# eichenberger/stereo-svo-slam

Measured on AMD Instinct MI355X. Metric: tracked_frames_per_sec, higher is better.
Workload: dtype f32

## Files before the change

### include/svo_hip.h

```cpp
#ifndef SVO_HIP_H
#define SVO_HIP_H

#include <stddef.h>

#include "svo_types.h"

#ifdef __cplusplus
extern "C" {
#endif

enum {
    SVO_OK = 0,
    SVO_ERR_INVALID = -1,
    SVO_ERR_HIP = -2,
    SVO_ERR_NO_DEVICE = -3,
    SVO_ERR_CAPACITY = -4
};

typedef struct svo_handle svo_handle;

const char *svo_last_error(void);
int svo_version(void);

int svo_handle_create(int device, int max_keypoints, svo_handle **out);
// ... 542 lines not shown
int svo_cloud_points(svo_handle *h, int n, const svo_cloud_src *src, const int64_t *first, const svo_cloud_style *style,
                     svo_map_point *points, int32_t *counts);

#define SVO_SNAPSHOT_MAGIC   0x534f5653u
#define SVO_SNAPSHOT_VERSION 1
#define SVO_SNAPSHOT_BYTE_ORDER 0x01020304u
enum { SVO_SNAPSHOT_COMPLETE = 0,
       SVO_SNAPSHOT_TOO_SMALL = 1 };

struct svo_snapshot_info {
    uint32_t magic, version, byte_order;
    uint32_t status;
    int64_t  host_bytes, data_bytes;
    svo_camera_settings cam;
    int32_t  width, height;
    int32_t  capacity;
    int32_t  pyramid_levels, lk_levels;
    int32_t  frame_id;
    int32_t  n_keypoints;
    int32_t  n_trajectory;
    int32_t  n_keyframes, keyframes_retired;
    int32_t  n_image_sets;
    int32_t  n_planes;
    int32_t  first_keyframe;
};
typedef struct svo_snapshot_keyframe {
    float   pose[6];
    int32_t n;
    int32_t image_set;
} svo_snapshot_keyframe;
typedef struct svo_snapshot_plane {
    int64_t offset;
    int32_t row_bytes, rows;
} svo_snapshot_plane;

typedef struct svo_snapshot {
    void   *host;  int64_t host_capacity;
    void   *data;  int64_t data_capacity;
} svo_snapshot;

int svo_snapshot_size(svo_ctx *ctx, int seq, int64_t *host_bytes, int64_t *data_bytes);
int svo_submit_save(svo_ctx *ctx, const int *seqs, int n, svo_snapshot *snaps, int mem);
int svo_save_sequences(svo_ctx *ctx, const int *seqs, int n, svo_snapshot *snaps, int mem);
int svo_submit_load(svo_ctx *ctx, const int *seqs, int n, const svo_snapshot *snaps, int mem);
int svo_load_sequences(svo_ctx *ctx, const int *seqs, int n, const svo_snapshot *snaps, int mem);
int svo_snapshot_info(const void *host_part, int64_t bytes, struct svo_snapshot_info *out);
typedef struct svo_copy_segment {
    const void *src;
    void       *dst;
    int64_t     row_bytes, rows;
    int64_t     src_pitch, dst_pitch;
} svo_copy_segment;
int svo_copy_segments(svo_handle *h, int n, const svo_copy_segment *segs);

typedef struct svo_frame_stats {
    int32_t frame_id;
    int32_t is_keyframe;
    int32_t n_keypoints;
    int32_t n_keyframes;
    int32_t inside_count;
    int32_t overflow;
    float   pose_sia[6];
    float   pose_refined[6];
    float   sia_cost, reproj_cost;
    float   sia_ms;
    float   stage_ms[8];
    svo_gn_trace sia_trace[SVO_MAX_PYRAMID_LEVELS];
    svo_gn_trace reproj_trace;
} svo_frame_stats;
int svo_get_frame_stats(svo_ctx *ctx, int seq, svo_frame_stats *out);
typedef struct svo_totals {
    int64_t frames;
    int64_t keyframes;
    int64_t keypoints;
    int64_t gn_gradient_calls;
    int64_t gn_cost_calls;
    double  stage_ms[8];
    double  wall_ms;
    int64_t launches;
    int32_t n_groups;
    int32_t image_sets;
} svo_totals;
int svo_get_totals(svo_ctx *ctx, svo_totals *out);
int svo_ctx_enable_timing(svo_ctx *ctx, int on);
int svo_ctx_set_fast_solver(svo_ctx *ctx, int on);
int svo_ctx_set_exact_pinv(svo_ctx *ctx, int on);

enum { SVO_KERNEL_SIA_GN = 0,
       SVO_KERNEL_REPROJ_GN = 1 };
typedef struct svo_launch_shape {
    int32_t kernel;
    int32_t waves;
    int32_t mode;
    int32_t cap;
    int64_t launches;
} svo_launch_shape;
int svo_ctx_get_launch_shapes(svo_ctx *ctx, svo_launch_shape *out, int max, int *n);
int svo_pick_launch_shapes(const svo_camera_settings *cam, int width, int height, int batch, int n_bound,
                           int rec_cap, int exact, svo_launch_shape out[2]);
int svo_pick_sia_lds_bytes(const svo_camera_settings *cam, int width, int height, int batch, int n_bound,
                           int rec_cap, int exact, int64_t *lds_bytes);

int svo_pinv6_check(svo_handle *h, const float *H_dev, int n, float *out_dev, int32_t *sweeps_dev, int impl);
int svo_solve6_check(svo_handle *h, const float *H_dev, const float *b_dev, int n, float *out_dev,
                     int32_t *sweeps_dev, int impl);
int svo_sia_records_check(svo_handle *h, int batch, int stride, const int32_t *n_dev, int n_bound,
                          const svo_kp2d *kps2d, const uint32_t *flags, const svo_image *prev_pyr,
                          const svo_camera_settings *cam, int rec_cap, uint32_t ws_fill, float *rec_out,
                          float *ref_out, int64_t *n_diff, int64_t *first_diff);
int svo_reproj_gn_batch(svo_handle *h, int batch, int stride, const int32_t *n_dev, int n_bound, svo_kp2d *kps2d,
                        const svo_kp3d *kps3d, uint32_t *flags, const svo_camera_settings *cam,
                        const svo_kp2d *tracked, const float *err, const float *pose_in, float *pose_out,
                        float *cost, svo_gn_trace *trace, int32_t *zero_out, int *waves, int *cap);
int svo_sparse_align_batch(svo_handle *h, int batch, int stride, const int32_t *n_dev, int n_bound,
                           const svo_kp2d *kps2d, const svo_kp3d *kps3d, const uint32_t *flags,
                           const svo_image *prev_pyr, const svo_image *cur_pyr, const svo_camera_settings *cam,
                           const float *pose_guess, int dbg_level, uint32_t ws_fill, float *pose_out, float *cost,
                           svo_gn_trace *trace, float *dbg, int *waves, int *mode, int *cap);
int svo_sparse_align_batch_mats(svo_handle *h, int batch, int stride, const int32_t *n_dev, int n_bound,
                                const svo_kp2d *kps2d, const svo_kp3d *kps3d, const uint32_t *flags,
                                const svo_image *prev_pyr, const svo_image *cur_pyr, const svo_camera_settings *cam,
                                const float *pose_guess, int dbg_level, uint32_t ws_fill, float *pose_out, float *cost,
                                svo_gn_trace *trace, float *dbg, int *waves, int *mode, int *cap, void *mats_out);
int svo_pose_mats_layout(int64_t *block_bytes, int64_t *rd_offset, int64_t *r_offset, int64_t *ri_offset,
                         int64_t *t_offset);
int svo_filter_update_batch(svo_handle *h, int batch, int stride, const int32_t *n_dev, int n_bound, svo_kp2d *kps2d,
                            svo_kp3d *kps3d, uint32_t *flags, const svo_camera_settings *cam,
                            const float *frame_pose, const float *disparity, const svo_kp3d *ref3d,
                            const svo_kp2d *ref2d, const float *kf_pose, int32_t *outlier_count,
                            int32_t *inlier_count, float *kf_inv_depth, float *kf_variance,
                            int do_outlier_check, int do_update, int do_flags, int do_reproject, int width,
                            int height, int32_t *inside_count);
typedef struct svo_klt_keyframe {
    svo_image lk[SVO_LK_LEVELS];
    int32_t n_lk;
    int32_t n_kps;
    const svo_kp2d *kps2d;
    void *tmpl;
    uint8_t *tmpl_valid;
    int64_t tmpl_bytes, tmpl_valid_bytes;
    int32_t tmpl_cap, tmpl_win;
} svo_klt_keyframe;
typedef struct svo_klt_sequence {
    const svo_klt_keyframe *kfs;
    int32_t n_kfs;
    int32_t n_cur;
    svo_image cur[SVO_LK_LEVELS];
    const int32_t *n;
    const int32_t *kf_id;
    const int32_t *kp_index;
    const svo_kp3d *kps3d;
    const float *pose;
    svo_camera_settings cam;
    svo_kp2d *tracked;
    uint8_t *status;
    float *err;
    svo_kp2d *proj_out;
    svo_kp2d *ref_out;
} svo_klt_sequence;
int svo_klt_track_batch(svo_handle *h, int batch, const svo_klt_sequence *seqs, int n_bound, int win, int use_mats);
int svo_klt_cache_layout(int win, int64_t *record_bytes, int64_t *header_offset, int64_t *header_bytes, int *levels);

typedef struct svo_kps_planes {
    svo_kp2d *kps2d;
    svo_kp3d *kps3d;
    uint32_t *flags;
    int32_t  *kf_id, *kp_index, *outlier_count, *inlier_count;
    float    *kf_inv_depth, *kf_variance, *score;
    int32_t  *level_type;
    uint32_t *color;
    int32_t  *n;
} svo_kps_planes;
int svo_keyframe_launch_info(int cap, int max_cells, int tmpl_cap, int *compact_threads, int *merge_threads,
                             int64_t *tmpl_valid_bytes);
typedef struct svo_compact_sequence {
    svo_kps_planes src, dst;
    int32_t mode, width, height, start;
    const int32_t *enable;
    int32_t *zero, *zero_res, *min_kf;
    int32_t zero_count, zero_res_count;
} svo_compact_sequence;
int svo_compact_batch(svo_handle *h, int batch, const svo_compact_sequence *seqs, int cap, int *threads);
typedef struct svo_merge_sequence {
    svo_camera_settings cam;
    int32_t width, height;
    const svo_det_cell *det;
    const int32_t *n_det;
    svo_kps_planes kps;
    svo_det_cell *sel;
    int32_t *sel_level, *sel_cell, *occupied;
    int32_t *old_count, *overflow;
    const int32_t *enable;
    int32_t occupied_count, pad_;
} svo_merge_sequence;
int svo_keyframe_merge_batch(svo_handle *h, int batch, const svo_merge_sequence *seqs, int n_levels, int max_cells,
                             int cap, int *threads);
typedef struct svo_kf_init_sequence {
    svo_camera_settings cam;
    int32_t first_frame, new_kf_id, kf_mask, evict_id;
    svo_kps_planes kps, record;
    const int32_t *old_count;
    const float *disparity, *frame_pose;
    void *kfs;
    int64_t kfs_bytes;
    uint32_t *color_lcg;
    int32_t *n_out;
    const int32_t *enable;
    void *tmpl;
    uint8_t *tmpl_valid;
    int32_t tmpl_valid_bytes, tmpl_cap, tmpl_win, pad_;
} svo_kf_init_sequence;
int svo_keyframe_init_batch(svo_handle *h, int batch, const svo_kf_init_sequence *seqs, int cap);
int svo_keyframe_record_layout(int64_t *record_bytes, int64_t *n_offset, int64_t *pose_offset, int64_t *tmpl_offset,
                               int64_t *tmpl_valid_offset, int64_t *tmpl_cap_offset, int64_t *tmpl_win_offset,
                               int64_t plane_offsets[12]);
typedef struct svo_ssd_sequence {
    svo_image left, right;
    const int32_t *n;
    const svo_kp2d *kps2d;
    float *disparity;
    int32_t win, search_x, search_y, clamp_half;
    int32_t first, cap;
    const int32_t *first_ptr;
    const int32_t *enable;
} svo_ssd_sequence;
int svo_ssd_disparity_batch(svo_handle *h, int batch, const svo_ssd_sequence *seqs, int n_bound, int win, int search_y,
                            int *max_win);

typedef struct svo_filter_keyframe {
    float pose[6];
    svo_kp2d *kps2d;
    svo_kp3d *kps3d;
    uint32_t *flags;
    int32_t *outlier_count, *inlier_count;
    int32_t n, pad_;
} svo_filter_keyframe;
typedef struct svo_filter_table_sequence {
    svo_camera_settings cam;
    svo_kps_planes kps;
    const float *frame_pose;
    const float *disparity;
    const svo_filter_keyframe *kfs;
    void *records;
    int64_t records_bytes;
    int32_t table, kf_mask, width, height;
    int32_t *inside_count;
} svo_filter_table_sequence;
int svo_filter_update_table_batch(svo_handle *h, int batch, const svo_filter_table_sequence *seqs, int n_bound,
                                  int do_outlier_check, int do_update, int do_flags, int do_reproject);

#ifdef __cplusplus
}
#endif
#endif
```

### stereo-svo-slam_amd/csrc/keyframe.hip

```cpp
#include "svo_kernels.hpp"
#include "svo_tracker.hpp"
#include <cstdlib>

namespace svo {

__device__ inline int block_exclusive_scan(int v, int* s_wave , int& total) {
    const int tid = threadIdx.x, lane = tid & 63, wave = tid >> 6;
    int inc = v;
#pragma unroll
    for (int o = 1; o < 64; o <<= 1) {
        const int t = __shfl_up(inc, o, 64);
        if (lane >= o) inc += t;
    }
    __syncthreads();
    if (lane == 63) s_wave[wave] = inc;
    __syncthreads();
    int base = 0, tot = 0;
    for (int w = 0; w < (int)(blockDim.x >> 6); w++) {
        const int x = s_wave[w];
        if (w < wave) base += x;
        tot += x;
    }
    total = tot;
    return base + inc - v;
}

__device__ inline void copy_kp(const KpsDev& d, int di, const KpsDev& s, int si) {
    G(d.kps2d)[di] = G(s.kps2d)[si];
    G(d.kps3d)[di] = G(s.kps3d)[si];
    G(d.flags)[di] = G(s.flags)[si];
    G(d.kf_id)[di] = G(s.kf_id)[si];
    G(d.kp_index)[di] = G(s.kp_index)[si];
    G(d.outl)[di] = G(s.outl)[si];
    G(d.inl)[di] = G(s.inl)[si];
    G(d.kfx)[di] = G(s.kfx)[si];
    G(d.kfP)[di] = G(s.kfP)[si];
    G(d.score)[di] = G(s.score)[si];
    G(d.level_type)[di] = G(s.level_type)[si];
    G(d.color)[di] = G(s.color)[si];
}

__global__ __launch_bounds__(1024) void compact_kernel(const CompactArgs* __restrict__ args) {
    const CompactArgs& a = args[blockIdx.x];
    if (a.enable && !*G(a.enable)) return;
    __shared__ int s_wave[16];
    __shared__ int s_min_kf;
    __shared__ unsigned s_live[2];
    const int tid = threadIdx.x;
    if (tid == 0) { s_min_kf = INT_MAX; s_live[0] = s_live[1] = 0u; }
    const int n = a.start ? 0 : *G(a.src.n);
    const int per = (n + (int)blockDim.x - 1) / (int)blockDim.x;
    const int i0 = tid * per, i1 = min(n, i0 + per);
    int cnt = 0;
    for (int i = i0; i < i1; i++) {
        const uint32_t f = G(a.src.flags)[i];
        bool keep;
        if (a.mode == 0) {
            keep = !(f & SVO_IGNORE_COMPLETELY);
        } else {
            const svo_kp2d k = G(a.src.kps2d)[i];
            keep = !((k.x < 0) || (k.y < 0) || (k.x > a.width) || (k.y > a.height) ||
                     (f & SVO_IGNORE_COMPLETELY) || (f & SVO_IGNORE_DURING_REFINEMENT));
        }
        cnt += keep ? 1 : 0;
    }
    int total;
    int pos = block_exclusive_scan(cnt, s_wave, total);
    int min_kf = INT_MAX;
    for (int i = i0; i < i1; i++) {
        const uint32_t f = G(a.src.flags)[i];
        bool keep;
        if (a.mode == 0) {
            keep = !(f & SVO_IGNORE_COMPLETELY);
        } else {
            const svo_kp2d k = G(a.src.kps2d)[i];
            keep = !((k.x < 0) || (k.y < 0) || (k.x > a.width) || (k.y > a.height) ||
                     (f & SVO_IGNORE_COMPLETELY) || (f & SVO_IGNORE_DURING_REFINEMENT));
        }
        if (keep) {
            copy_kp(a.dst, pos++, a.src, i);
            min_kf = min(min_kf, G(a.src.kf_id)[i]);
        }
    }
    if (tid == 0) {
        *G(a.dst.n) = total;
        if (a.start) *G(a.src.n) = 0;
    }
    if (a.min_kf) {
        if (min_kf != INT_MAX) atomicMin(&s_min_kf, min_kf);
        __syncthreads();
        const int base = s_min_kf;
        for (int i = i0; i < i1; i++) {
            if (G(a.src.flags)[i] & SVO_IGNORE_COMPLETELY) continue;
            const int j = G(a.src.kf_id)[i] - base;
            if (j >= 0 && j < 64) atomicOr(&s_live[j >> 5], 1u << (j & 31));
        }
        __syncthreads();
        if (tid == 0) { G(a.min_kf)[0] = base; G(a.min_kf)[1] = (int)s_live[0]; G(a.min_kf)[2] = (int)s_live[1]; }
    }
    if (a.zero)
        for (int i = tid; i < a.zero_count; i += blockDim.x) G(a.zero)[i] = 0;
    if (a.zero_res)
        for (int i = tid; i < a.zero_res_count; i += blockDim.x) G(a.zero_res)[i] = 0;
}

int compact_pick_threads(int cap) {
    static const int env_threads = getenv("SVO_COMPACT_THREADS") ? atoi(getenv("SVO_COMPACT_THREADS")) : 0;
    return env_threads >= 64 && env_threads <= 1024 && env_threads % 64 == 0 ? env_threads : (cap <= 1024 ? 256 : 1024);
}
void launch_compact(const CompactArgs* d_args, int batch, int cap, hipStream_t stream) {
    hipLaunchKernelGGL(compact_kernel, dim3(batch), dim3(compact_pick_threads(cap)), 0, stream, d_args);
}

constexpr int DET_MAX_CW = 96, DET_MAX_CH = 64;

__constant__ int c_ring_dx[16] = {0, 1, 2, 3, 3, 3, 2, 1, 0, -1, -2, -3, -3, -3, -2, -1};
__constant__ int c_ring_dy[16] = {3, 3, 2, 1, 0, -1, -2, -3, -3, -3, -2, -1, 0, 1, 2, 3};

__device__ inline bool fast_is_corner(const uint8_t* p, int stride, int threshold) {
    const int v = p[0];
    const int lo = v - threshold, hi = v + threshold;
    unsigned md = 0, mb = 0;
#pragma unroll
    for (int k = 0; k < 16; k++) {
        const int q = p[c_ring_dy[k] * stride + c_ring_dx[k]];
        md = __builtin_amdgcn_alignbit(md, (unsigned)(q - lo), 31);
        mb = __builtin_amdgcn_alignbit(mb, (unsigned)(hi - q), 31);
    }
    auto run9 = [](unsigned m) {
        const unsigned w = m | (m << 16);
        unsigned r = w & (w >> 1);
        r &= r >> 2;
        r &= r >> 4;
        return (r & (w >> 8)) != 0;
    };
    return run9(md) || run9(mb);
}
__device__ inline int fast_corner_score(const uint8_t* p, int stride, int threshold) {
    int d[25];
    const int v = p[0];
#pragma unroll
    for (int k = 0; k < 25; k++) d[k] = v - (int)p[c_ring_dy[k & 15] * stride + c_ring_dx[k & 15]];
    int pmin[12], pmax[12];
#pragma unroll
    for (int j = 0; j < 12; j++) { pmin[j] = min(d[2 * j + 1], d[2 * j + 2]); pmax[j] = max(d[2 * j + 1], d[2 * j + 2]); }
    int a0 = threshold;
#pragma unroll
    for (int k = 0; k < 16; k += 2) {
        const int j = k >> 1;
        const int a = min(min(min(pmin[j], pmin[j + 1]), pmin[j + 2]), pmin[j + 3]);
        a0 = max(max(a0, min(a, d[k])), min(a, d[k + 9]));
    }
    int b0 = -a0;
#pragma unroll
    for (int k = 0; k < 16; k += 2) {
        const int j = k >> 1;
        const int b = max(max(max(pmax[j], pmax[j + 1]), pmax[j + 2]), pmax[j + 3]);
        b0 = min(min(b0, max(b, d[k])), max(b, d[k + 9]));
    }
    return -b0 - 1;
}

struct SmallDiv {
    unsigned m;
    int d;
    __device__ explicit SmallDiv(int d_) : m(((1u << 20) + (unsigned)d_ - 1u) / (unsigned)d_), d(d_) {}
    __device__ int quot(int i) const { return (int)(((unsigned)i * m) >> 20); }
    __device__ void divmod(int i, int& q, int& r) const { q = quot(i); r = i - q * d; }
};


template <int CW, int CH, int DET_LIST>
__global__ __launch_bounds__(256) void kf_detect_kernel(const DetectArgs* __restrict__ args) {
    constexpr int DET_TW = ((CW + 8 + 3 + 3) & ~3), DET_TH = CH + 8;
    constexpr int DET_RW = CW + 2, DET_RH = CH + 2;
    const DetectArgs& a = args[blockIdx.z];
    if (a.enable && !*G(a.enable)) return;
    const int level = blockIdx.y;
    if (level >= a.n_levels) return;
    const ImgView im = a.level[level];
    const int gw = a.grid_w >> level, gh = a.grid_h >> level;
    if (gw <= 0 || gh <= 0 || gw > CW || gh > CH) return;
    const int ncx = im.w / gw, ncy = max(im.h / gh, 1);
    const int cell = blockIdx.x;
    if (cell >= ncx * ncy) return;
    const int cxi = cell % ncx, cyi = cell / ncx;
    const int left = cxi * gw, top = cyi * gh;
    const int tid = threadIdx.x;

    __shared__ __attribute__((aligned(16))) uint8_t s_t[DET_TH * DET_TW];
    __shared__ uint8_t s_raw[DET_RH * DET_RW];
    __shared__ unsigned s_key[4];
    __shared__ uint16_t s_list[DET_LIST];
    __shared__ int s_nlist;

    const int tw = gw + 8, th = gh + 8;
    const SmallDiv div_tw(tw), div_rw(gw + 2), div_gw(gw), div_gh(gh);
    const int x0 = (left - 4) & ~3, ox = (left - 4) - x0;
    const bool inside = left - 4 >= 0 && top - 4 >= 0 && left + gw + 4 <= im.w && top + gh + 4 <= im.h && x0 + ((ox + tw + 3) & ~3) <= im.stride &&
                        (((reinterpret_cast<uintptr_t>(im.data) | (uintptr_t)im.stride) & 3) == 0);
    const uint8_t* const s_tb = s_t + (inside ? ox : 0);
    if (inside) {
        const int nq = (ox + tw + 3) >> 2;
        const SmallDiv div_nq(nq);
        SVO_GP(const uint8_t) g0 = im.g() + (size_t)(top - 4) * im.stride + x0;
        for (int i = tid; i < nq * th; i += 256) {
            int r, c;
            div_nq.divmod(i, r, c);
            *reinterpret_cast<uint32_t*>(&s_t[r * DET_TW + 4 * c]) = *reinterpret_cast<SVO_GP(const uint32_t)>(g0 + r * im.stride + 4 * c);
        }
    } else {
        for (int i = tid; i < tw * th; i += 256) {
            int r, c;
            div_tw.divmod(i, r, c);
            const int gy = reflect101(top - 4 + r, im.h), gx = reflect101(left - 4 + c, im.w);
            s_t[r * DET_TW + c] = im.g()[(size_t)gy * im.stride + gx];
        }
    }
    __syncthreads();
    const int rw = gw + 2, rh = gh + 2;
    if (tid == 0) s_nlist = 0;
    __syncthreads();
    for (int i = tid; i < rw * rh; i += 256) {
        int r, c;
        div_rw.divmod(i, r, c);
        const int gy = top - 1 + r, gx = left - 1 + c;
        int sc = 0;
        if (gx >= 3 && gx < im.w - 3 && gy >= 3 && gy < im.h - 3 &&
            fast_is_corner(&s_tb[(r + 3) * DET_TW + c + 3], DET_TW, 6)) {
            const int slot = atomicAdd(&s_nlist, 1);
            if (slot < DET_LIST) s_list[slot] = (uint16_t)i;
            else sc = fast_corner_score(&s_tb[(r + 3) * DET_TW + c + 3], DET_TW, 6);
        }
        s_raw[r * DET_RW + c] = (uint8_t)sc;
    }
    __syncthreads();
    {
        const int nl = min(s_nlist, DET_LIST);
        for (int q = tid; q < nl; q += 256) {
            const int i = s_list[q];
            int r, c;
            div_rw.divmod(i, r, c);
            s_raw[r * DET_RW + c] = (uint8_t)fast_corner_score(&s_tb[(r + 3) * DET_TW + c + 3], DET_TW, 6);
        }
    }
    __syncthreads();
    unsigned best = 0;
    for (int i = tid; i < gw * gh; i += 256) {
        int r, c;
        div_gw.divmod(i, r, c);
        if (top + r >= im.h) continue;
        const uint8_t* q = &s_raw[(r + 1) * DET_RW + c + 1];
        const int sc = q[0];
        if (sc && sc > q[1] && sc > q[-1] && sc > q[-DET_RW - 1] && sc > q[-DET_RW] &&
            sc > q[-DET_RW + 1] && sc > q[DET_RW - 1] && sc > q[DET_RW] && sc > q[DET_RW + 1]) {
            const unsigned key = ((unsigned)sc << 20) | (0xFFFFFu - (unsigned)i);
            best = max(best, key);
        }
    }
#pragma unroll
    for (int o = 32; o >= 1; o >>= 1) best = max(best, (unsigned)__shfl_xor((int)best, o, 64));
    if ((tid & 63) == 0) s_key[tid >> 6] = best;
    __syncthreads();
    best = max(max(s_key[0], s_key[1]), max(s_key[2], s_key[3]));
    int type = SVO_KP_FAST;
    float score, px, py;
    if (best) {
        const int i = (int)(0xFFFFFu - (best & 0xFFFFFu));
        score = (float)(best >> 20);
        px = (float)(left + i % gw);
        py = (float)(top + i / gw);
    } else {
        __syncthreads();
        unsigned eb = 0;
        for (int i = tid; i < gw * gh; i += 256) {
            int c, r;
            div_gh.divmod(i, c, r);
            const uint8_t* p1 = &s_tb[(r + 4) * DET_TW + c + 4];
            const uint8_t* p0 = p1 - DET_TW;
            const uint8_t* p2 = p1 + DET_TW;
            int v = (p0[1] - p0[-1]) + 2 * (p1[1] - p1[-1]) + (p2[1] - p2[-1]);
            v = v < 0 ? 0 : (v > 255 ? 255 : v);
            const unsigned key = ((unsigned)v << 20) | (0xFFFFFu - (unsigned)i);
            eb = max(eb, key);
        }
#pragma unroll
        for (int o = 32; o >= 1; o >>= 1) eb = max(eb, (unsigned)__shfl_xor((int)eb, o, 64));
        if ((tid & 63) == 0) s_key[tid >> 6] = eb;
        __syncthreads();
        eb = max(max(s_key[0], s_key[1]), max(s_key[2], s_key[3]));
        const int i = (int)(0xFFFFFu - (eb & 0xFFFFFu));
        score = (float)(eb >> 20);
        px = (float)(left + i / gh);
        py = (float)(top + i % gh);
        type = SVO_KP_EDGELET;
    }
    if (tid == 0) {
        DetCell o;
        o.x = px; o.y = py; o.score = score; o.type = type;
        G(a.out)[(size_t)level * a.max_cells + cell] = o;
        if (cell == 0) G(a.n_out)[level] = ncx * ncy;
    }
}

constexpr DetectShape DET_SMALL = {56, 48, 1024}, DET_LARGE = {DET_MAX_CW, DET_MAX_CH, 2048};

DetectShape detect_pick_shape(int grid_w, int grid_h) {
    return grid_w <= DET_SMALL.cell_w && grid_h <= DET_SMALL.cell_h ? DET_SMALL : DET_LARGE;
}

void launch_detect(const DetectArgs* d_args, int batch, int max_cells, int n_levels, int grid_w, int grid_h, hipStream_t stream) {
    if (detect_pick_shape(grid_w, grid_h).cell_w == DET_SMALL.cell_w)
        hipLaunchKernelGGL((kf_detect_kernel<DET_SMALL.cell_w, DET_SMALL.cell_h, DET_SMALL.list>), dim3(max_cells, n_levels, batch), dim3(256), 0, stream, d_args);
    else
        hipLaunchKernelGGL((kf_detect_kernel<DET_LARGE.cell_w, DET_LARGE.cell_h, DET_LARGE.list>), dim3(max_cells, n_levels, batch), dim3(256), 0, stream, d_args);
}

__global__ __launch_bounds__(1024) void kf_select_merge_kernel(const MergeArgs* __restrict__ args) {
    const MergeArgs& a = args[blockIdx.x];
    if (a.enable && !*G(a.enable)) return;
    const int tid = threadIdx.x, nthr = blockDim.x;
    const int nsel = G(a.n_det)[0];
    const int n_old = *G(a.kps.n);
    const int mcw = a.cam.grid_height, mch = a.cam.grid_width;
    const int ncx = (a.width + mcw - 1) / mcw, ncy = (a.height + mch - 1) / mch;
    const int ncells = ncx * ncy;

    for (int j = tid; j < nsel; j += nthr) {
        DetCell s = G(a.det)[j];
        int lvl = 0;
        for (int i = 1; i < a.n_levels; i++) {
            if (j >= G(a.n_det)[i]) continue;
            const DetCell c = G(a.det)[(size_t)i * a.max_cells + j];
            if (s.type == SVO_KP_FAST && c.type == SVO_KP_EDGELET) continue;
            if (s.type == c.type && s.score > c.score) continue;
            s = c;
            s.x *= (float)(1 << i);
            s.y *= (float)(1 << i);
            lvl = i;
        }
        G(a.sel)[j] = s;
        G(a.sel_level)[j] = lvl;
        G(a.sel_cell)[j] = -1;
    }
    for (int c = tid; c < ncells; c += nthr) G(a.occupied)[c] = 0;
    __syncthreads();
    for (int i = tid; i < n_old; i += nthr) {
        const svo_kp2d k = G(a.kps.kps2d)[i];
        if (!(k.x > 0 && k.y > 0)) continue;
        const int xi = (int)floorf(k.x) / mcw, yi = (int)floorf(k.y) / mch;
        if (xi >= ncx || yi >= ncy) continue;
        const int l = xi * mcw, t = yi * mch;
        if (k.x > l && k.x < l + mcw && k.y > t && k.y < t + mch) G(a.occupied)[xi * ncy + yi] = 1;
    }
    __syncthreads();
    for (int j = tid; j < nsel; j += nthr) {
        const DetCell s = G(a.sel)[j];
        if (!(s.x > 0 && s.y > 0)) continue;
        const int xi = (int)floorf(s.x) / mcw, yi = (int)floorf(s.y) / mch;
        if (xi >= ncx || yi >= ncy) continue;
        const int l = xi * mcw, t = yi * mch;
        if (s.x > l && s.x < l + mcw && s.y > t && s.y < t + mch && !G(a.occupied)[xi * ncy + yi])
            G(a.sel_cell)[j] = xi * ncy + yi;
    }
    __syncthreads();
    __shared__ int s_cnt;
    if (tid == 0) s_cnt = 0;
    __syncthreads();
    for (int j = tid; j < nsel; j += nthr) {
        const int cj = G(a.sel_cell)[j];
        if (cj < 0) continue;
        int pos = 0;
        for (int q = 0; q < nsel; q++) {
            const int cq = G(a.sel_cell)[q];
            pos += (cq >= 0 && (cq < cj || (cq == cj && q < j))) ? 1 : 0;
        }
        atomicAdd(&s_cnt, 1);
        const int di = n_old + pos;
        if (di < a.cap) {
            const DetCell s = G(a.sel)[j];
            G(a.kps.kps2d)[di] = svo_kp2d{s.x, s.y};
            G(a.kps.score)[di] = s.score;
            G(a.kps.level_type)[di] = G(a.sel_level)[j] | (s.type << 8);
        }
    }
    __syncthreads();
    if (tid == 0) {
        int n_new = s_cnt;
        if (n_old + n_new > a.cap) { n_new = a.cap - n_old; *G(a.overflow) = 1; }
        *G(a.old_count) = n_old;
        *G(a.kps.n) = n_old + n_new;
    }
}

int select_merge_pick_threads(int max_cells) {
    static const int env_threads = getenv("SVO_MERGE_THREADS") ? atoi(getenv("SVO_MERGE_THREADS")) : 0;
    return env_threads >= 64 && env_threads <= 1024 && env_threads % 64 == 0 ? env_threads : (max_cells <= 512 ? 256 : 1024);
}
void launch_select_merge(const MergeArgs* d_args, int batch, int max_cells, hipStream_t stream) {
    hipLaunchKernelGGL(kf_select_merge_kernel, dim3(batch), dim3(select_merge_pick_threads(max_cells)), 0, stream, d_args);
}

__global__ __launch_bounds__(256) void kf_init_kernel(const KfInitArgs* __restrict__ args) {
    const KfInitArgs& a = args[blockIdx.x];
    if (a.enable && !*G(a.enable)) return;
    const int tid = threadIdx.x;
    const int n = *G(a.kps.n), old_count = *G(a.old_count);
    __shared__ PoseMats pm;
    __shared__ int s_cnt[4];
    float pose[6];
    for (int i = 0; i < 6; i++) pose[i] = a.first_frame ? 0.f : G(a.frame_pose)[i];
    if (tid == 0) {
        pose_mats(pose, pm);
        G(a.kfs)[a.new_kf_id & a.kf_mask] = a.record;
        if (a.evict_id >= 0) G(a.kfs)[a.evict_id & a.kf_mask].tmpl = nullptr;
    }
    if (a.record.tmpl_valid)
        for (int i = tid; i < a.tmpl_valid_bytes / 4; i += 256) ((SVO_GP(uint32_t))a.record.tmpl_valid)[i] = 0u;
    __syncthreads();
    const float fx = a.cam.fx, fy = a.cam.fy, cx = a.cam.cx, cy = a.cam.cy, baseline = a.cam.baseline;
    const uint32_t lcg0 = a.first_frame ? SVO_COLOR_LCG_SEED : *G(a.color_lcg);
    for (int i = old_count + tid; i < n; i += 256) {
        const svo_kp2d kp = G(a.kps.kps2d)[i];
        const float disparity = G(a.disparity)[i];
        float loc[3];
        kp_triangulate(kp.x, kp.y, disparity, fx, fy, cx, cy, baseline, loc);
        const float _z = loc[2];
        G(a.kps.kps3d)[i] = kp_to_world(pm, loc);
        uint32_t st = lcg0;
        for (int q = old_count; q <= i; q++) st = st * 1664525u + 1013904223u;
        G(a.kps.color)[i] = (st >> 8) & 0xFFFFFFu;
        G(a.kps.kf_id)[i] = a.new_kf_id;
        G(a.kps.kp_index)[i] = i;
        G(a.kps.flags)[i] = SVO_IGNORE_TEMPORARY;
        G(a.kps.inl)[i] = 0;
        G(a.kps.outl)[i] = 0;
        const float deviation = (float)(0.5 / (double)(baseline / fx));
        G(a.kps.kfP)[i] = deviation * deviation;
        G(a.kps.kfx)[i] = 1 / _z;
    }
    __syncthreads();
    const KfDev& kf = a.record;
    int not_temp = 0;
    for (int i = tid; i < n; i += 256) {
        const uint32_t f = G(a.kps.flags)[i];
        G(kf.kps2d)[i] = G(a.kps.kps2d)[i];
        G(kf.kps3d)[i] = G(a.kps.kps3d)[i];
        G(kf.flags)[i] = f;
        G(kf.outlier_count)[i] = G(a.kps.outl)[i];
        G(kf.inlier_count)[i] = G(a.kps.inl)[i];
        G(kf.kf_id)[i] = G(a.kps.kf_id)[i];
        G(kf.kp_index)[i] = G(a.kps.kp_index)[i];
        G(kf.score)[i] = G(a.kps.score)[i];
        G(kf.level_type)[i] = G(a.kps.level_type)[i];
        G(kf.color)[i] = G(a.kps.color)[i];
        G(kf.kfx)[i] = G(a.kps.kfx)[i];
        G(kf.kfP)[i] = G(a.kps.kfP)[i];
        not_temp += (f & SVO_IGNORE_TEMPORARY) ? 0 : 1;
// ... 25 lines not shown
```

### stereo-svo-slam_amd/csrc/svo_capi.hip

```cpp
#include <hip/hip_runtime.h>

#include <algorithm>
#include <cstring>
#include <memory>
#include <new>

#include "svo_handle.hpp"

using namespace svo;

extern "C" const char* svo_last_error(void) { return svo_error_text; }
extern "C" int svo_version(void) { return 100; }

extern "C" int svo_handle_create(int device, int max_keypoints, svo_handle** out) {
    if (!out || max_keypoints <= 0) return svo_set_error(SVO_ERR_INVALID, "svo_handle_create: bad arguments");
    int count = 0;
    if (hipGetDeviceCount(&count) != hipSuccess || count <= 0)
        return svo_set_error(SVO_ERR_NO_DEVICE, "no HIP device visible: libsvo_hip has no CPU fallback");
    if (device < 0 || device >= count) return svo_set_error(SVO_ERR_INVALID, "device %d out of range", device);
    HIP_TRY(hipSetDevice(device));
    std::unique_ptr<svo_handle> h(new (std::nothrow) svo_handle());
    if (!h) return svo_set_error(SVO_ERR_INVALID, "out of host memory");
    h->device = device;
    h->max_kps = max_keypoints;
// ... 206 lines not shown
extern "C" int svo_reproj_gn(svo_handle* h, svo_kp2d* kps2d, const svo_kp3d* kps3d, uint32_t* flags,
                             int n, const svo_camera_settings* cam, const svo_kp2d* tracked,
                             const float* err, const float* pose_in, float* pose_out, float* cost,
                             svo_gn_trace* trace) {
    CHECK_H(h);
    if (!cam || !pose_in || !pose_out || n < 0) return svo_set_error(SVO_ERR_INVALID, "svo_reproj_gn: bad arguments");
    ReprojArgs ra;
    memset(&ra, 0, sizeof(ra));
    ra.cam = *cam;
    int* d_n;
    int rc = stage_n(h, n, &d_n);
    if (rc) return rc;
    ra.n_ptr = d_n;
    ra.kps2d = kps2d; ra.kps3d = kps3d; ra.flags = flags; ra.tracked = tracked; ra.err = err;
    ra.pose_in = pose_in; ra.pose_out = pose_out; ra.cost_out = cost; ra.trace = trace;
    ra.exact_pinv = h->exact_pinv;
    ReprojArgs* d;
    rc = stage(h, ra, &d);
    if (rc) return rc;
    const LaunchStatus reproj_launch = launch_reproj(d, 1, n, h->stream);
    HIP_TRY(reproj_launch.err);
    if (!reproj_launch.shape.fits) return svo_set_error(SVO_ERR_CAPACITY, "svo_reproj_gn: %d keypoints do not fit LDS", n);
    HIP_TRY(hipGetLastError());
    return SVO_OK;
}

extern "C" int svo_ssd_disparity(svo_handle* h, const svo_image* left, const svo_image* right,
                                 const svo_kp2d* kps2d, int n, int win, int search_x, int search_y,
                                 int clamp_half, float* disparity) {
    CHECK_H(h);
    if (!left || !right || n < 0) return svo_set_error(SVO_ERR_INVALID, "svo_ssd_disparity: bad arguments");
    if (win < 1 || win > 35 || search_x < 0 || search_x > 64 || search_y < 0 || search_y > 8)
        return svo_set_error(SVO_ERR_INVALID, "svo_ssd_disparity: win<=35, search_x<=64, search_y<=8 supported");
    SsdArgs sa;
    memset(&sa, 0, sizeof(sa));
    sa.left = make_view(*left); sa.right = make_view(*right);
    int* d_n;
    int rc = stage_n(h, n, &d_n);
    if (rc) return rc;
    sa.n_ptr = d_n; sa.kps2d = kps2d; sa.disparity = disparity;
    sa.win = win; sa.search_x = search_x; sa.search_y = search_y; sa.clamp_half = clamp_half;
    sa.first = 0;
    SsdArgs* d;
    rc = stage(h, sa, &d);
    if (rc) return rc;
    launch_ssd(d, 1, n, win, search_y, h->stream);
    HIP_TRY(hipGetLastError());
    return SVO_OK;
}

extern "C" int svo_depth_filter_update(svo_handle* h, const svo_kp2d* kps2d, svo_kp3d* kps3d,
                                       const uint32_t* flags, int n, const svo_camera_settings* cam,
                                       const float* frame_pose, const float* disparity,
                                       const svo_kp3d* ref3d, const svo_kp2d* ref2d,
                                       const float* kf_pose, int32_t* outlier_count,
                                       int32_t* inlier_count, float* kf_inv_depth, float* kf_variance,
                                       int do_outlier_check, int do_update) {
    CHECK_H(h);
    if (!cam || !frame_pose || !kf_pose || n < 0)
        return svo_set_error(SVO_ERR_INVALID, "svo_depth_filter_update: bad arguments");
    FilterArgs fa;
    memset(&fa, 0, sizeof(fa));
    fa.cam = *cam;
    int* d_n;
    int rc = stage_n(h, n, &d_n);
    if (rc) return rc;
    fa.n_ptr = d_n;
    fa.frame_pose = frame_pose;
    fa.kps2d = const_cast<svo_kp2d*>(kps2d);
    fa.kps3d = kps3d;
    fa.flags = const_cast<uint32_t*>(flags);
    fa.outlier_count = outlier_count; fa.inlier_count = inlier_count;
    fa.kf_inv_depth = kf_inv_depth; fa.kf_variance = kf_variance;
    fa.disparity = disparity; fa.ref3d = ref3d; fa.ref2d = ref2d; fa.kf_pose = kf_pose;
    fa.do_outlier_check = do_outlier_check; fa.do_update = do_update;
    FilterArgs* d;
    rc = stage(h, fa, &d);
    if (rc) return rc;
    launch_filter(d, 1, n, h->stream);
    HIP_TRY(hipGetLastError());
    return SVO_OK;
}

static int check_detect_levels(const char* who, int n_levels, int grid_width, int grid_height) {
    if (n_levels < 1 || n_levels > SVO_MAX_PYRAMID_LEVELS)
        return svo_set_error(SVO_ERR_INVALID, "%s: n_levels must be 1..%d", who, SVO_MAX_PYRAMID_LEVELS);
    if (grid_width < 4 || grid_height < 4 || grid_width > 96 || grid_height > 64)
        return svo_set_error(SVO_ERR_INVALID, "%s: grid cell must be within 4..96 x 4..64", who);
    if ((grid_width >> (n_levels - 1)) == 0 || (grid_height >> (n_levels - 1)) == 0)
        return svo_set_error(SVO_ERR_INVALID, "%s: the cell of level %d is empty", who, n_levels - 1);
    return SVO_OK;
}
static int detect_level_cells(const char* who, int l, int width, int height, int grid_width, int grid_height, int* cells) {
    const int gw = grid_width >> l, gh = grid_height >> l;
    if (width < 1 || height < gh)
        return svo_set_error(SVO_ERR_INVALID, "%s: level %d (%d x %d) is lower than its cell (%d x %d)", who, l, width, height, gw, gh);
    *cells = (width / gw) * (height / gh);
    return SVO_OK;
}

extern "C" int svo_detect_shape(int width, int height, int n_levels, int grid_width, int grid_height, int* max_cells,
                                int* cell_width, int* cell_height, int* list_capacity) {
    int rc = check_detect_levels("svo_detect_shape", n_levels, grid_width, grid_height);
    if (rc) return rc;
    int most = 1;
    for (int l = 0; l < n_levels; l++) {
        int nc;
        if ((rc = detect_level_cells("svo_detect_shape", l, width >> l, height >> l, grid_width, grid_height, &nc))) return rc;
        most = std::max(most, nc);
    }
    const DetectShape s = detect_pick_shape(grid_width, grid_height);
    if (max_cells) *max_cells = most;
    if (cell_width) *cell_width = s.cell_w;
    if (cell_height) *cell_height = s.cell_h;
    if (list_capacity) *list_capacity = s.list;
    return SVO_OK;
}

static_assert(sizeof(svo_det_cell) == sizeof(DetCell) && offsetof(svo_det_cell, score) == offsetof(DetCell, score) &&
              offsetof(svo_det_cell, type) == offsetof(DetCell, type), "svo_det_cell is the kernel's DetCell");

extern "C" int svo_detect_keypoints(svo_handle* h, int n_levels, const svo_image* levels, int grid_width, int grid_height,
                                    int max_cells, svo_det_cell* cells, int32_t* counts) {
    CHECK_H(h);
    if (!levels || !cells || !counts || max_cells < 1)
        return svo_set_error(SVO_ERR_INVALID, "svo_detect_keypoints: bad arguments");
    int rc = check_detect_levels("svo_detect_keypoints", n_levels, grid_width, grid_height);
    if (rc) return rc;
    DetectArgs da;
    memset(&da, 0, sizeof(da));
    for (int l = 0; l < n_levels; l++) {
        if (!levels[l].data || levels[l].stride < levels[l].width)
            return svo_set_error(SVO_ERR_INVALID, "svo_detect_keypoints: level %d: no data or stride < width", l);
        int nc;
        if ((rc = detect_level_cells("svo_detect_keypoints", l, levels[l].width, levels[l].height, grid_width, grid_height, &nc)))
            return rc;
        if (nc > max_cells)
            return svo_set_error(SVO_ERR_CAPACITY, "svo_detect_keypoints: level %d has %d cells, max_cells = %d", l, nc, max_cells);
        da.level[l] = make_view(levels[l]);
    }
    da.n_levels = n_levels; da.grid_w = grid_width; da.grid_h = grid_height;
    da.out = reinterpret_cast<DetCell*>(cells); da.n_out = counts; da.max_cells = max_cells;
    HIP_TRY(hipMemsetAsync(counts, 0, sizeof(int32_t) * (size_t)n_levels, h->stream));
    DetectArgs* d;
    rc = stage(h, da, &d);
    if (rc) return rc;
    launch_detect(d, 1, max_cells, n_levels, grid_width, grid_height, h->stream);
    HIP_TRY(hipGetLastError());
    return SVO_OK;
}
```

### stereo-svo-slam_amd/csrc/svo_capi_check.hip

```cpp
#include <hip/hip_runtime.h>

#include <algorithm>
#include <climits>
#include <cstring>
#include <vector>

#include "svo_handle.hpp"

using namespace svo;

static bool bad_batch(int batch, const void* seqs) { return batch < 1 || batch > 4096 || !seqs; }

extern "C" int svo_pick_launch_shapes(const svo_camera_settings* cam, int width, int height, int batch, int n_bound,
                                      int rec_cap, int exact, svo_launch_shape out[2]) {
    if (!cam || !out || width < 1 || height < 1 || batch < 1)
        return svo_set_error(SVO_ERR_INVALID, "svo_pick_launch_shapes: bad arguments");
    const LaunchShape s = sia_pick_shape(batch, *cam, width, height, n_bound, rec_cap, exact);
    const LaunchShape r = reproj_pick_shape(batch, n_bound);
    out[0] = {SVO_KERNEL_SIA_GN, s.waves, s.mode, s.cap, s.fits ? 1 : 0};
    out[1] = {SVO_KERNEL_REPROJ_GN, r.waves, r.mode, r.cap, r.fits ? 1 : 0};
    return SVO_OK;
}

extern "C" int svo_pick_sia_lds_bytes(const svo_camera_settings* cam, int width, int height, int batch, int n_bound,
// ... 508 lines not shown
        if (n < 0 || n > n_bound)
            return svo_set_error(SVO_ERR_INVALID, "svo_klt_track_batch: sequence %d: n = %d is outside 0..n_bound = %d", b, n, n_bound);
        idx.resize((size_t)n); ids.assign((size_t)n, 0);
        if (n > 0) {
            HIP_TRY(hipMemcpy(idx.data(), s.kp_index, sizeof(int32_t) * (size_t)n, hipMemcpyDeviceToHost));
            if (s.kf_id) HIP_TRY(hipMemcpy(ids.data(), s.kf_id, sizeof(int32_t) * (size_t)n, hipMemcpyDeviceToHost));
        }
        for (int i = 0; i < n; i++)
            if (ids[(size_t)i] < 0 || ids[(size_t)i] >= s.n_kfs || idx[(size_t)i] < 0 || idx[(size_t)i] >= s.kfs[ids[(size_t)i]].n_kps)
                return svo_set_error(SVO_ERR_INVALID, "svo_klt_track_batch: sequence %d point %d: keyframe %d, index %d", b, i,
                                     ids[(size_t)i], idx[(size_t)i]);
    }
    KfDev* d_table;
    int rc = stage(h, table, &d_table);
    if (rc) return rc;
    DevPtr<PoseMats> mats;
    if (use_mats) {
        std::vector<const float*> poses((size_t)batch);
        for (int b = 0; b < batch; b++) poses[(size_t)b] = seqs[b].pose;
        const float** d_poses;
        rc = stage(h, poses, &d_poses);
        if (rc) return rc;
        HIP_TRY(dev_malloc(mats, sizeof(PoseMats) * (size_t)batch));
        klt_pose_mats_kernel<<<batch, 1, 0, h->stream>>>(d_poses, mats.get());
        HIP_TRY(hipGetLastError());
    }
    std::vector<KltArgs> blocks((size_t)batch);
    for (int b = 0; b < batch; b++) {
        const svo_klt_sequence& s = seqs[b];
        KltArgs& ka = blocks[(size_t)b];
        memset(&ka, 0, sizeof(ka));
        ka.kfs = d_table + first_kf[(size_t)b]; ka.kf_mask = -1; ka.kf_id = s.kf_id; ka.n_cur = s.n_cur;
        for (int l = 0; l < s.n_cur; l++) ka.cur[l] = make_view(s.cur[l]);
        ka.n_ptr = s.n; ka.prev_pts = nullptr; ka.cur_pts = s.tracked; ka.status = s.status;
        ka.err = s.err; ka.win = win;
        ka.proj_pose = s.pose; ka.proj_mats = use_mats ? mats.get() + b : nullptr; ka.kps3d = s.kps3d; ka.proj_out = s.proj_out;
        ka.kp_index = s.kp_index; ka.ref_out = s.ref_out; ka.cam = s.cam;
    }
    KltArgs* d;
    rc = stage(h, blocks, &d);
    if (rc) { (void)hipStreamSynchronize(h->stream); return rc; }
    launch_klt(d, batch, n_bound, win, h->stream);
    return finish_launch(h);
}

extern "C" int svo_klt_cache_layout(int win, int64_t* record_bytes, int64_t* header_offset, int64_t* header_bytes, int* levels) {
    if (win < 3 || win > 35) return svo_set_error(SVO_ERR_INVALID, "svo_klt_cache_layout: window must be 3..35");
    if (record_bytes) *record_bytes = (int64_t)klt_template_bytes(win);
    if (header_offset) *header_offset = (int64_t)klt_template_header_offset(win);
    if (header_bytes) *header_bytes = (int64_t)klt_template_header_bytes();
    if (levels) *levels = SVO_LK_LEVELS;
    return SVO_OK;
}

static_assert(sizeof(svo_kps_planes) == 104 && sizeof(svo_compact_sequence) == 264 && sizeof(svo_merge_sequence) == 272 &&
              sizeof(svo_kf_init_sequence) == 400 && sizeof(svo_ssd_sequence) == 112, "the layouts the Python binding restates");

static KpsDev kps_dev(const svo_kps_planes& p) {
    KpsDev k;
    k.kps2d = p.kps2d; k.kps3d = p.kps3d; k.flags = p.flags; k.kf_id = p.kf_id; k.kp_index = p.kp_index;
    k.outl = p.outlier_count; k.inl = p.inlier_count; k.kfx = p.kf_inv_depth; k.kfP = p.kf_variance;
    k.score = p.score; k.level_type = p.level_type; k.color = p.color; k.n = p.n;
    return k;
}
static bool planes_missing(const svo_kps_planes& p, bool need_n) {
    return !p.kps2d || !p.kps3d || !p.flags || !p.kf_id || !p.kp_index || !p.outlier_count || !p.inlier_count ||
           !p.kf_inv_depth || !p.kf_variance || !p.score || !p.level_type || !p.color || (need_n && !p.n);
}
static int read_i32(const int32_t* dev, int count, int32_t* out) {
    HIP_TRY(hipMemcpy(out, dev, sizeof(int32_t) * (size_t)count, hipMemcpyDeviceToHost));
    return SVO_OK;
}

extern "C" int svo_keyframe_launch_info(int cap, int max_cells, int tmpl_cap, int* compact_threads, int* merge_threads,
                                        int64_t* tmpl_valid_bytes) {
    if (cap < 1 || max_cells < 1 || tmpl_cap < 0)
        return svo_set_error(SVO_ERR_INVALID, "svo_keyframe_launch_info: need cap >= 1, max_cells >= 1, tmpl_cap >= 0");
    if (compact_threads) *compact_threads = compact_pick_threads(cap);
    if (merge_threads) *merge_threads = select_merge_pick_threads(max_cells);
    if (tmpl_valid_bytes) *tmpl_valid_bytes = (int64_t)kf_tmpl_valid_bytes(tmpl_cap);
    return SVO_OK;
}

extern "C" int svo_compact_batch(svo_handle* h, int batch, const svo_compact_sequence* seqs, int cap, int* threads) {
    CHECK_H(h);
    if (bad_batch(batch, seqs) || cap < 1)
        return svo_set_error(SVO_ERR_INVALID, "svo_compact_batch: need 1 <= batch <= 4096, seqs and cap >= 1");
    HIP_TRY(hipStreamSynchronize(h->stream));
    std::vector<CompactArgs> blocks((size_t)batch);
    for (int b = 0; b < batch; b++) {
        const svo_compact_sequence& s = seqs[b];
        if (planes_missing(s.src, true) || planes_missing(s.dst, true) || (s.mode != 0 && s.mode != 1) ||
            (s.start != 0 && s.start != 1) || s.zero_count < 0 || s.zero_res_count < 0 || (s.zero_count > 0 && !s.zero) ||
            (s.zero_res_count > 0 && !s.zero_res))
            return svo_set_error(SVO_ERR_INVALID, "svo_compact_batch: sequence %d: bad arguments", b);
        if (s.min_kf && s.mode != 0)
            return svo_set_error(SVO_ERR_INVALID, "svo_compact_batch: sequence %d: min_kf is defined for mode 0 only", b);
        if (!s.start) {
            int32_t n = 0;
            if (const int rc = read_i32(s.src.n, 1, &n)) return rc;
            if (n < 0 || n > cap)
                return svo_set_error(SVO_ERR_INVALID, "svo_compact_batch: sequence %d: n = %d is outside 0..cap = %d", b, n, cap);
        }
        CompactArgs& ca = blocks[(size_t)b];
        memset(&ca, 0, sizeof(ca));
        ca.src = kps_dev(s.src); ca.dst = kps_dev(s.dst); ca.mode = s.mode;
        ca.width = s.width; ca.height = s.height;
        ca.enable = s.enable;
        ca.zero = s.zero; ca.zero_count = s.zero_count;
        ca.start = s.start;
        ca.zero_res = s.zero_res; ca.zero_res_count = s.zero_res_count;
        ca.min_kf = s.min_kf;
    }
    CompactArgs* d;
    const int rc = stage(h, blocks, &d);
    if (rc) return rc;
    if (threads) *threads = compact_pick_threads(cap);
    launch_compact(d, batch, cap, h->stream);
    return finish_launch(h);
}

extern "C" int svo_keyframe_merge_batch(svo_handle* h, int batch, const svo_merge_sequence* seqs, int n_levels,
                                        int max_cells, int cap, int* threads) {
    CHECK_H(h);
    if (bad_batch(batch, seqs) || n_levels < 1 || n_levels > SVO_MAX_PYRAMID_LEVELS || max_cells < 1 || cap < 1)
        return svo_set_error(SVO_ERR_INVALID, "svo_keyframe_merge_batch: need 1 <= batch <= 4096, seqs, n_levels 1..%d, "
                             "max_cells >= 1 and cap >= 1", SVO_MAX_PYRAMID_LEVELS);
    HIP_TRY(hipStreamSynchronize(h->stream));
    std::vector<MergeArgs> blocks((size_t)batch);
    for (int b = 0; b < batch; b++) {
        const svo_merge_sequence& s = seqs[b];
        if (planes_missing(s.kps, true) || !s.det || !s.n_det || !s.sel || !s.sel_level || !s.sel_cell || !s.occupied ||
            !s.old_count || !s.overflow || s.width < 1 || s.height < 1 || s.cam.grid_width < 1 || s.cam.grid_height < 1)
            return svo_set_error(SVO_ERR_INVALID, "svo_keyframe_merge_batch: sequence %d: bad arguments", b);
        const int64_t cells = ((int64_t)(s.width + s.cam.grid_height - 1) / s.cam.grid_height) *
                              ((int64_t)(s.height + s.cam.grid_width - 1) / s.cam.grid_width);
        if (cells > s.occupied_count)
            return svo_set_error(SVO_ERR_INVALID, "svo_keyframe_merge_batch: sequence %d: %lld merge cells, occupied holds %d", b,
                                 (long long)cells, s.occupied_count);
        int32_t nd[SVO_MAX_PYRAMID_LEVELS], n = 0;
        if (const int rc = read_i32(s.n_det, n_levels, nd)) return rc;
        if (const int rc = read_i32(s.kps.n, 1, &n)) return rc;
        for (int l = 0; l < n_levels; l++)
            if (nd[l] < 0 || nd[l] > max_cells)
                return svo_set_error(SVO_ERR_INVALID, "svo_keyframe_merge_batch: sequence %d: n_det[%d] = %d is outside "
                                     "0..max_cells = %d", b, l, nd[l], max_cells);
        if (n < 0 || n > cap)
            return svo_set_error(SVO_ERR_INVALID, "svo_keyframe_merge_batch: sequence %d: n = %d is outside 0..cap = %d", b, n, cap);
        MergeArgs& ma = blocks[(size_t)b];
        memset(&ma, 0, sizeof(ma));
        ma.cam = s.cam; ma.width = s.width; ma.height = s.height;
        ma.det = reinterpret_cast<const DetCell*>(s.det); ma.n_det = s.n_det; ma.n_levels = n_levels; ma.max_cells = max_cells;
        ma.kps = kps_dev(s.kps); ma.cap = cap;
        ma.sel = reinterpret_cast<DetCell*>(s.sel); ma.sel_level = s.sel_level; ma.sel_cell = s.sel_cell; ma.occupied = s.occupied;
        ma.old_count = s.old_count; ma.overflow = s.overflow;
        ma.enable = s.enable;
    }
    MergeArgs* d;
    const int rc = stage(h, blocks, &d);
    if (rc) return rc;
    if (threads) *threads = select_merge_pick_threads(max_cells);
    launch_select_merge(d, batch, max_cells, h->stream);
    return finish_launch(h);
}

extern "C" int svo_keyframe_record_layout(int64_t* record_bytes, int64_t* n_offset, int64_t* pose_offset, int64_t* tmpl_offset,
                                          int64_t* tmpl_valid_offset, int64_t* tmpl_cap_offset, int64_t* tmpl_win_offset,
                                          int64_t plane_offsets[12]) {
    if (record_bytes) *record_bytes = (int64_t)sizeof(KfDev);
    if (n_offset) *n_offset = (int64_t)offsetof(KfDev, n);
    if (pose_offset) *pose_offset = (int64_t)offsetof(KfDev, pose);
    if (tmpl_offset) *tmpl_offset = (int64_t)offsetof(KfDev, tmpl);
    if (tmpl_valid_offset) *tmpl_valid_offset = (int64_t)offsetof(KfDev, tmpl_valid);
    if (tmpl_cap_offset) *tmpl_cap_offset = (int64_t)offsetof(KfDev, tmpl_cap);
    if (tmpl_win_offset) *tmpl_win_offset = (int64_t)offsetof(KfDev, tmpl_win);
    if (plane_offsets) {
        const size_t o[12] = {offsetof(KfDev, kps2d), offsetof(KfDev, kps3d), offsetof(KfDev, flags), offsetof(KfDev, kf_id),
                              offsetof(KfDev, kp_index), offsetof(KfDev, outlier_count), offsetof(KfDev, inlier_count),
                              offsetof(KfDev, kfx), offsetof(KfDev, kfP), offsetof(KfDev, score), offsetof(KfDev, level_type),
                              offsetof(KfDev, color)};
        for (int i = 0; i < 12; i++) plane_offsets[i] = (int64_t)o[i];
    }
    return SVO_OK;
}

extern "C" int svo_keyframe_init_batch(svo_handle* h, int batch, const svo_kf_init_sequence* seqs, int cap) {
    CHECK_H(h);
    if (bad_batch(batch, seqs) || cap < 1)
        return svo_set_error(SVO_ERR_INVALID, "svo_keyframe_init_batch: need 1 <= batch <= 4096, seqs and cap >= 1");
    HIP_TRY(hipStreamSynchronize(h->stream));
    std::vector<KfInitArgs> blocks((size_t)batch);
    for (int b = 0; b < batch; b++) {
        const svo_kf_init_sequence& s = seqs[b];
        if (planes_missing(s.kps, true) || planes_missing(s.record, false) || !s.old_count || !s.disparity || !s.kfs ||
            !s.color_lcg || !s.n_out || (!s.first_frame && !s.frame_pose) || (s.first_frame != 0 && s.first_frame != 1) ||
            s.new_kf_id < 0 || s.evict_id < -1)
            return svo_set_error(SVO_ERR_INVALID, "svo_keyframe_init_batch: sequence %d: bad arguments", b);
        if (s.kf_mask < 0 || s.kf_mask > (1 << 20) || ((s.kf_mask + 1) & s.kf_mask) != 0 ||
            (int64_t)(s.kf_mask + 1) * (int64_t)sizeof(KfDev) > s.kfs_bytes || (reinterpret_cast<uintptr_t>(s.kfs) & 7))
            return svo_set_error(SVO_ERR_INVALID, "svo_keyframe_init_batch: sequence %d: the table needs kf_mask + 1 = a power "
                                 "of two records of %zu bytes, 8-byte aligned", b, sizeof(KfDev));
        if (s.tmpl_valid_bytes < 0 || s.tmpl_valid_bytes % 4 != 0 || (s.tmpl_valid_bytes > 0 && !s.tmpl_valid) ||
            (reinterpret_cast<uintptr_t>(s.tmpl_valid) & 3))
            return svo_set_error(SVO_ERR_INVALID, "svo_keyframe_init_batch: sequence %d: tmpl_valid must be 4-byte aligned and "
                                 "tmpl_valid_bytes a multiple of 4", b);
        int32_t n = 0, old_count = 0;
        if (const int rc = read_i32(s.kps.n, 1, &n)) return rc;
        if (const int rc = read_i32(s.old_count, 1, &old_count)) return rc;
        if (n < 0 || n > cap || old_count < 0 || old_count > n)
            return svo_set_error(SVO_ERR_INVALID, "svo_keyframe_init_batch: sequence %d: need 0 <= old_count = %d <= n = %d <= "
                                 "cap = %d", b, old_count, n, cap);
        KfInitArgs& ia = blocks[(size_t)b];
        memset(&ia, 0, sizeof(ia));
        ia.cam = s.cam; ia.kps = kps_dev(s.kps); ia.old_count = s.old_count;
        ia.disparity = s.disparity; ia.frame_pose = s.frame_pose;
        ia.first_frame = s.first_frame; ia.new_kf_id = s.new_kf_id; ia.kfs = static_cast<KfDev*>(s.kfs); ia.kf_mask = s.kf_mask;
        ia.color_lcg = s.color_lcg; ia.n_out = s.n_out;
        ia.enable = s.enable;
        KfDev& r = ia.record;
        r.kps2d = s.record.kps2d; r.kps3d = s.record.kps3d; r.flags = s.record.flags;
        r.outlier_count = s.record.outlier_count; r.inlier_count = s.record.inlier_count;
        r.kf_id = s.record.kf_id; r.kp_index = s.record.kp_index; r.score = s.record.score;
        r.level_type = s.record.level_type; r.color = s.record.color; r.kfx = s.record.kf_inv_depth; r.kfP = s.record.kf_variance;
        r.tmpl = s.tmpl; r.tmpl_valid = s.tmpl_valid; r.tmpl_cap = s.tmpl_cap; r.tmpl_win = s.tmpl_win;
        ia.tmpl_valid_bytes = s.tmpl_valid_bytes;
        ia.evict_id = s.evict_id;
    }
    KfInitArgs* d;
    const int rc = stage(h, blocks, &d);
    if (rc) return rc;
    launch_kf_init(d, batch, h->stream);
    return finish_launch(h);
}

extern "C" int svo_ssd_disparity_batch(svo_handle* h, int batch, const svo_ssd_sequence* seqs, int n_bound, int win,
                                       int search_y, int* max_win) {
    CHECK_H(h);
    constexpr int kMaxIndex = 1 << 29;
    if (bad_batch(batch, seqs) || n_bound < 0 || n_bound > kMaxIndex)
        return svo_set_error(SVO_ERR_INVALID, "svo_ssd_disparity_batch: need 1 <= batch <= 4096, seqs and 0 <= n_bound <= 2^29");
    if (win < 1 || win > 35 || search_y < 0 || search_y > 8)
        return svo_set_error(SVO_ERR_INVALID, "svo_ssd_disparity_batch: win<=35, search_y<=8 supported");
    HIP_TRY(hipStreamSynchronize(h->stream));
    std::vector<SsdArgs> blocks((size_t)batch);
    for (int b = 0; b < batch; b++) {
// ... 99 lines not shown
```

### stereo-svo-slam_amd/csrc/svo_ctx.hip

```cpp
#include <hip/hip_runtime.h>

#include <algorithm>
#include <atomic>
#include <climits>
#include <cmath>
#include <condition_variable>
#include <cstdlib>
#include <cstring>
#include <deque>
#include <memory>
#include <mutex>
#include <new>
#include <string>
#include <thread>
#include <vector>

#include "svo_group.hpp"
#include "svo_group_state.hpp"
#include "svo_host.hpp"
#include "svo_kernels.hpp"

struct svo_ctx {
    struct Export {
        int what = 0, mem = 0;
// ... 1122 lines not shown
    return SVO_OK;
}

extern "C" int svo_ctx_assign_rigs(svo_ctx* c, const int* seqs, const int* rigs, int n) {
    if (!c || n < 0 || (n > 0 && (!seqs || !rigs))) return svo_set_error(SVO_ERR_INVALID, "svo_ctx_assign_rigs: bad arguments");
    for (int i = 0; i < n; i++) {
        if (seqs[i] < 0 || seqs[i] >= c->B)
            return svo_set_error(SVO_ERR_INVALID, "svo_ctx_assign_rigs: sequence %d out of range", seqs[i]);
        if (!rig_exists(c, rigs[i])) return svo_set_error(SVO_ERR_INVALID, "svo_ctx_assign_rigs: rig %d does not exist", rigs[i]);
    }
    if (c->failed.load()) return reject_failed(c, "svo_ctx_assign_rigs");
    const size_t map_bytes = svo::remap_map_bytes(c->width, c->height);
    for (auto& wp : c->workers) {
        svo_ctx::Worker& w = *wp;
        svo_ctx::Job job;
        for (int i = 0; i < n; i++) {
            if (seqs[i] < w.first || seqs[i] >= w.first + w.count) continue;
            const svo_ctx::Rig& r = c->rigs[rigs[i]];
            const uint8_t* base = r.maps.get();
            job.assign.push_back(seqs[i] - w.first);
            job.bindings.push_back(RigBinding{rigs[i], r.cam, {base, base ? base + map_bytes : nullptr}});
        }
        if (!job.assign.empty()) worker_submit(w, std::move(job));
    }
    for (int i = 0; i < n; i++) c->slot_rig[seqs[i]] = rigs[i];
    return SVO_OK;
}

extern "C" int svo_ctx_get_slot_rig(svo_ctx* c, int seq, int* rig, svo_camera_settings* cam) {
    if (!c || seq < 0 || seq >= c->B) return svo_set_error(SVO_ERR_INVALID, "bad ctx / sequence index");
    const int rc = ctx_drain(c);
    if (rc) return rc;
    if (rig) *rig = c->slot_rig[seq];
    if (cam) *cam = c->rigs[c->slot_rig[seq]].cam;
    return SVO_OK;
}

extern "C" int svo_ctx_get_rigs(svo_ctx* c, int* n, int64_t* map_bytes) {
    if (!c) return svo_set_error(SVO_ERR_INVALID, "svo_ctx_get_rigs: bad ctx");
    const int rc = ctx_drain(c);
    if (rc) return rc;
    if (n) *n = (int)std::count_if(c->rigs.begin(), c->rigs.end(), [](const svo_ctx::Rig& r) { return r.used; });
    if (map_bytes) *map_bytes = (int64_t)c->rig_map_bytes();
    return SVO_OK;
}

extern "C" int svo_ctx_set_exact_pinv(svo_ctx* c, int on);
extern "C" int svo_ctx_set_fast_solver(svo_ctx* c, int on) { return svo_ctx_set_exact_pinv(c, on == 0); }

extern "C" int svo_ctx_set_exact_pinv(svo_ctx* c, int on) {
    if (!c) return svo_set_error(SVO_ERR_INVALID, "bad ctx");
    const int rc = ctx_drain(c);
    if (!rc)
        for (auto& w : c->workers) grp_set_exact_pinv(w->g.get(), on);
    return rc;
}

extern "C" int svo_ctx_enable_timing(svo_ctx* c, int on) {
    if (!c) return svo_set_error(SVO_ERR_INVALID, "bad ctx");
    const int rc = ctx_drain(c);
    if (!rc)
        for (auto& w : c->workers) grp_enable_timing(w->g.get(), on);
    return rc;
}

extern "C" int svo_get_totals(svo_ctx* c, svo_totals* out) {
    if (!c || !out) return svo_set_error(SVO_ERR_INVALID, "svo_get_totals: bad arguments");
    const int rc = ctx_drain(c);
    if (rc) return rc;
    std::memset(out, 0, sizeof(*out));
    for (auto& w : c->workers) {
        const svo_totals t = grp_totals(w->g.get());
        out->frames += t.frames; out->keyframes += t.keyframes; out->keypoints += t.keypoints;
        out->gn_gradient_calls += t.gn_gradient_calls; out->gn_cost_calls += t.gn_cost_calls;
        for (int i = 0; i < 8; i++) out->stage_ms[i] += t.stage_ms[i];
        out->wall_ms = std::max(out->wall_ms, t.wall_ms);
        out->launches += t.launches;
        out->image_sets += t.image_sets;
    }
    out->n_groups = (int)c->workers.size();
    return SVO_OK;
}

extern "C" int svo_ctx_get_launch_shapes(svo_ctx* c, svo_launch_shape* out, int max, int* n) {
    if (!c || !n || max < 0 || (max > 0 && !out)) return svo_set_error(SVO_ERR_INVALID, "svo_ctx_get_launch_shapes: bad arguments");
    const int rc = ctx_drain(c);
    if (rc) return rc;
    std::vector<svo_launch_shape> all;
    for (auto& w : c->workers)
        for (const svo_launch_shape& e : grp_launch_shapes(w->g.get())) {
            auto it = std::find_if(all.begin(), all.end(), [&e](const svo_launch_shape& a) {
                return a.kernel == e.kernel && a.waves == e.waves && a.mode == e.mode && a.cap == e.cap;
            });
            if (it == all.end()) all.push_back(e);
            else it->launches += e.launches;
        }
    std::sort(all.begin(), all.end(), [](const svo_launch_shape& a, const svo_launch_shape& b) {
        if (a.kernel != b.kernel) return a.kernel < b.kernel;
        if (a.waves != b.waves) return a.waves < b.waves;
        if (a.mode != b.mode) return a.mode < b.mode;
        return a.cap < b.cap;
    });
    *n = (int)all.size();
    for (int i = 0; i < std::min(max, *n); i++) out[i] = all[i];
    return SVO_OK;
}


static int fetch_info(int n, const svo::KpsDev& k, svo_kp2d* kps2d, svo_kp3d* kps3d, svo_kp_info* info) {
    if (n <= 0) return SVO_OK;
    if (kps2d) HIP_TRY(hipMemcpy(kps2d, k.kps2d, sizeof(svo_kp2d) * n, hipMemcpyDeviceToHost));
    if (kps3d) HIP_TRY(hipMemcpy(kps3d, k.kps3d, sizeof(svo_kp3d) * n, hipMemcpyDeviceToHost));
    if (!info) return SVO_OK;
    std::vector<uint32_t> fl(n), col(n);
    std::vector<int> kf(n), ki(n), ou(n), in(n), lt(n);
    std::vector<float> kx(n), kP(n), sc(n);
    const struct { void* dst; const void* src; } arrays[] = {
        {fl.data(), k.flags}, {ou.data(), k.outl}, {in.data(), k.inl}, {kf.data(), k.kf_id}, {ki.data(), k.kp_index},
        {kx.data(), k.kfx}, {kP.data(), k.kfP}, {sc.data(), k.score}, {lt.data(), k.level_type}, {col.data(), k.color}};
    for (const auto& a : arrays) HIP_TRY(hipMemcpy(a.dst, a.src, sizeof(uint32_t) * n, hipMemcpyDeviceToHost));
    for (int i = 0; i < n; i++) {
        svo_kp_info& o = svo::clear(info[i]);
        o.score = sc[i]; o.level = lt[i] & 0xff; o.type = (lt[i] >> 8) & 0xff;
        o.keyframe_id = kf[i]; o.keypoint_index = ki[i];
        o.color[0] = col[i] & 0xff; o.color[1] = (col[i] >> 8) & 0xff; o.color[2] = (col[i] >> 16) & 0xff;
        o.ignore_during_refinement = (fl[i] & SVO_IGNORE_DURING_REFINEMENT) != 0;
        o.ignore_completely = (fl[i] & SVO_IGNORE_COMPLETELY) != 0;
        o.ignore_temporary = (fl[i] & SVO_IGNORE_TEMPORARY) != 0;
        o.outlier_count = ou[i]; o.inlier_count = in[i];
        o.kf_inv_depth = kx[i]; o.kf_variance = kP[i];
    }
    return SVO_OK;
}

extern "C" int svo_get_pose(svo_ctx* ctx, int seq, float pose[6]) {
    svo_group* c; int s;
    if (const int rc = ctx_seq(ctx, seq, &c, &s)) return rc;
    svo::flush_pending(c);
    std::memcpy(pose, c->seqs[s].pose, sizeof(float) * 6);
    return SVO_OK;
}

extern "C" int svo_get_frame_keypoints(svo_ctx* ctx, int seq, svo_kp2d* kps2d, svo_kp3d* kps3d,
                                       svo_kp_info* info, int cap, int* n) {
    svo_group* c; int s;
    if (const int rc = ctx_seq(ctx, seq, &c, &s)) return rc;
    const svo::Seq& q = c->seqs[s];
    if (n) *n = q.n_host;
    return fetch_info(std::min(cap, q.n_host), q.kps[q.cur], kps2d, kps3d, info);
}

extern "C" int svo_get_keyframe_count(svo_ctx* ctx, int seq, int* count) {
    svo_group* c; int s;
    if (const int rc = ctx_seq(ctx, seq, &c, &s)) return rc;
    if (count) *count = (int)c->seqs[s].kfs.size();
    return SVO_OK;
}

extern "C" int svo_get_keyframe(svo_ctx* ctx, int seq, int id, svo_kp2d* kps2d, svo_kp3d* kps3d,
                                svo_kp_info* info, float pose[6], int cap, int* n) {
    svo_group* c; int s;
    if (const int rc = ctx_seq(ctx, seq, &c, &s)) return rc;
    const svo::Seq& q = c->seqs[s];
    if (id < 0 || id >= (int)q.kfs.size()) return svo_set_error(SVO_ERR_INVALID, "keyframe %d does not exist", id);
    if (id < q.kfs.first()) return svo_set_error(SVO_ERR_INVALID, "keyframe %d was trimmed", id);
    const svo::KfHost& k = q.kfs[id];
// ... 56 lines not shown
```

### stereo-svo-slam_amd/csrc/svo_group.hip

```cpp
#include <hip/hip_runtime.h>

#include <algorithm>
#include <cstdio>
#include <cstdlib>
#include <cstring>
#include <memory>
#include <new>
#include <vector>

#include "svo_group_state.hpp"

using namespace svo;

void GroupDelete::operator()(svo_group* c) const {
    (void)hipSetDevice(c->device);
    if (c->stream) (void)hipStreamSynchronize(c->stream.get());
    if (std::getenv("SVO_HOST_TIMING") && c->host_steps > 0) {
        static const char* names[7] = {"args", "launch", "pose_filter", "wait_frame", "kf_enqueue", "wait_kf", "bookkeeping"};
        std::fprintf(stderr, "[svo host ms/step over %ld steps]", c->host_steps);
        for (int i = 0; i < 7; i++) std::fprintf(stderr, " %s=%.3f", names[i], c->host_ms[i] / c->host_steps);
        std::fprintf(stderr, "\n");
    }
    delete c;
}
// ... 173 lines not shown
        w = (w + 1) / 2; h = (h + 1) / 2;
        if (w <= cam.window_size_opt_flow || h <= cam.window_size_opt_flow) return l + 1;
    }
    return SVO_LK_LEVELS;
}


static void size_group(svo_group* c) {
    const svo_camera_settings& cam = c->cam;
    const int width = c->width, height = c->height;
    c->cap = keypoint_capacity(cam, width, height);
    c->rec_cap = (int)align_up((size_t)c->cap, 512);
    c->max_kf = MAX_KEYFRAMES;
    if (const char* e = std::getenv("SVO_KEYFRAME_TABLE")) {
        const int t = std::atoi(e);
        if (t >= 4 && t <= MAX_KEYFRAMES && (t & (t - 1)) == 0) c->max_kf = t;
    }
    if (const char* e = std::getenv("SVO_KEEP_KEYFRAME_IMAGES")) c->retire_kf_images = std::atoi(e) == 0;
    c->n_lk = usable_lk_levels(cam, width, height);
    c->det_levels = cam.max_pyramid_levels / 2;
    c->max_cells = 1;
    for (int l = 0; l < c->det_levels; l++) {
        const int gw = cam.grid_width >> l, gh = cam.grid_height >> l;
        if (gw <= 0 || gh <= 0) { c->det_levels = l; break; }
        const int nc = ((width >> l) / gw) * std::max((height >> l) / gh, 1);
        c->max_cells = std::max(c->max_cells, nc);
    }
    c->merge_cells = ((width + cam.grid_height - 1) / cam.grid_height) *
                     ((height + cam.grid_width - 1) / cam.grid_width);
    c->set_layout = image_set_layout(c);
}

static int alloc_blocks(svo_group* c) {
    ArgBlocks& a = c->args;
    const size_t B = c->B;
    size_t off = 0;
    auto size = [&](auto& arr) { off += align_up(sizeof(typename std::decay_t<decltype(arr)>::type) * B, 256); };
    a.frame_arrays(size);
    a.frame_bytes = off;
    a.rig_arrays(size);
    a.frame_rig_bytes = off;
    a.keyframe_arrays(size);
    a.bytes = off;
    HIP_TRY(pinned_malloc(a.host, a.bytes));
    std::memset(a.host.get(), 0, a.bytes);
    int rc;
    if ((rc = dev_alloc(c, &a.dev, a.bytes))) return rc;
    off = 0;
    auto place = [&](auto& arr) {
        using T = typename std::decay_t<decltype(arr)>::type;
        arr.h = reinterpret_cast<T*>(a.host.get() + off);
        arr.d = reinterpret_cast<T*>(a.dev + off);
        off += align_up(sizeof(T) * B, 256);
    };
    a.frame_arrays(place);
    a.rig_arrays(place);
    a.keyframe_arrays(place);

    const size_t res_bytes = sizeof(FrameResult) * B, n_bytes = sizeof(int) * 2 * B, in_bytes = sizeof(int) * B;
    c->readback_bytes = res_bytes + n_bytes;
    uint8_t* db = nullptr;
    HIP_TRY(pinned_malloc(c->readback_host, res_bytes + n_bytes + in_bytes));
    uint8_t* hb = c->readback_host.get();
    std::memset(hb, 0, res_bytes + n_bytes + in_bytes);
    if ((rc = dev_alloc(c, &db, res_bytes + n_bytes + in_bytes))) return rc;
    c->h_res = reinterpret_cast<FrameResult*>(hb); c->d_res = reinterpret_cast<FrameResult*>(db);
    c->h_n = reinterpret_cast<int*>(hb + res_bytes); c->d_n_all = reinterpret_cast<int*>(db + res_bytes);
    c->h_inside = reinterpret_cast<int*>(hb + res_bytes + n_bytes);
    c->d_inside = reinterpret_cast<int*>(db + res_bytes + n_bytes);
    return SVO_OK;
}

static int alloc_sequence(svo_group* c, Seq& q, int s) {
    q.d_n = c->d_n_all + 2 * s;
    int rc = alloc_kps(c, q.kps[0], q.d_n);
    if (!rc) rc = alloc_kps(c, q.kps[1], q.d_n + 1);
    auto alloc = [&](auto** p, size_t count) { if (!rc) rc = dev_alloc(c, p, count); };
    const size_t cap = c->cap, cells = c->max_cells;
    alloc(&q.tracked, cap); alloc(&q.klt_err, cap); alloc(&q.klt_status, cap); alloc(&q.disparity, cap);
    alloc(&q.sia_rec, sia_rec_ws_floats(c->cam, c->rec_cap)); alloc(&q.sia_kpws, (size_t)9 * c->rec_cap);
    alloc(&q.sia_mats, 1); alloc(&q.d_kfs, c->max_kf);
    alloc(&q.det, SVO_MAX_PYRAMID_LEVELS * cells); alloc(&q.n_det, SVO_MAX_PYRAMID_LEVELS);
    alloc(&q.sel, cells); alloc(&q.sel_level, cells); alloc(&q.sel_cell, cells); alloc(&q.occupied, c->merge_cells);
    alloc(&q.color_lcg, 1);
    if (rc) return rc;
    q.kf.init();
    std::memset(&q.stats, 0, sizeof(q.stats));
    for (int i = 0; i < 4; i++)
        if ((rc = new_image_set(c, q))) return rc;
    return SVO_OK;
}

static int alloc_template_cache(svo_group* c) {
    const int B = c->B;
    const int cells = (c->width / c->cam.grid_width) * (c->height / c->cam.grid_height);
    c->tmpl_cap = std::min(c->cap, cells + 64);
    c->tmpl_block_bytes = align_up((size_t)c->tmpl_cap * SVO_LK_LEVELS * klt_template_bytes(c->cam.window_size_opt_flow), 256);
    int K = c->tmpl_block_bytes <= ((size_t)8 << 20) ? 8 : 4;
    if (const char* e = std::getenv("SVO_KLT_CACHE_KF")) K = std::max(0, std::min(std::atoi(e), 64));
    c->tmpl_valid_bytes = kf_tmpl_valid_bytes(c->tmpl_cap);
    size_t free_b = 0, total_b = 0;
    HIP_TRY(hipMemGetInfo(&free_b, &total_b));
    while (K > 0 && (size_t)B * K * c->tmpl_block_bytes > free_b / 3) K--;
    c->tmpl_kf = K;
    if (K == 0) return SVO_OK;
    uint8_t* base = nullptr; uint8_t* vbase = nullptr;
    int rc;
    if ((rc = dev_alloc(c, &base, (size_t)B * K * c->tmpl_block_bytes, false))) return rc;
    if ((rc = dev_alloc(c, &vbase, (size_t)B * K * c->tmpl_valid_bytes))) return rc;
    for (int s = 0; s < B; s++) {
        c->seqs[s].tmpl_base = base + (size_t)s * K * c->tmpl_block_bytes;
        c->seqs[s].tmpl_valid = vbase + (size_t)s * K * c->tmpl_valid_bytes;
    }
    return SVO_OK;
}

template <typename T>
static int alloc_mirrored_table(svo_group* c, ArgArray<T>& table, PinnedPtr<T>& host, size_t n) {
    PinnedPtr<T> pinned;
    HIP_TRY(pinned_malloc(pinned, sizeof(T) * n));
    T* dev = nullptr;
    if (const int rc = dev_alloc(c, &dev, n)) return rc;
    host = std::move(pinned);
    table.h = host.get();
    table.d = dev;
    return SVO_OK;
}

}

int grp_create(const svo_camera_settings* cam, int width, int height, int n_sequences, int device, Group* out) {
    int rc = check_settings(cam, width, height, n_sequences);
    if (rc) return rc;
    int count = 0;
    if (hipGetDeviceCount(&count) != hipSuccess || count <= 0)
        return svo_set_error(SVO_ERR_NO_DEVICE, "no HIP device visible: libsvo_hip has no CPU fallback");
    if (device < 0 || device >= count) return svo_set_error(SVO_ERR_INVALID, "device %d out of range", device);
    HIP_TRY(hipSetDevice(device));
    Group g(new (std::nothrow) svo_group());
    svo_group* c = g.get();
    if (!c) return svo_set_error(SVO_ERR_INVALID, "out of host memory");
    c->fmt = ingest_format(SVO_INPUT_GRAY_PAIR);
    c->device = device; c->B = n_sequences; c->width = width; c->height = height; c->cam = *cam;
    std::memset(&c->totals, 0, sizeof(c->totals));
    HIP_TRY(make_stream(c->stream));
    size_group(c);
    if ((rc = alloc_blocks(c))) return rc;
    for (Event& e : c->ev) HIP_TRY(make_event(e));
    c->seqs.resize(n_sequences);
    for (Seq& q : c->seqs) q.cam = c->cam;
    if ((rc = grow_set_slabs(c, 4 * n_sequences))) return rc;
    for (int s = 0; s < n_sequences; s++)
        if ((rc = alloc_sequence(c, c->seqs[s], s))) return rc;
    if ((rc = grow_kf_slabs(c, std::max(2 * n_sequences, 32)))) return rc;
    if ((rc = alloc_template_cache(c))) return rc;
    if ((rc = alloc_mirrored_table(c, c->remap_img, c->remap_img_host, 2 * (size_t)n_sequences))) return rc;
    HIP_TRY(hipDeviceSynchronize());
    *out = std::move(g);
    return SVO_OK;
}

void grp_set_exact_pinv(svo_group* c, int on) { c->exact_pinv = on != 0; }
void grp_set_rectification(svo_group* c, const RemapMap* maps) { c->rect = maps; }
void grp_enable_timing(svo_group* c, int on) { c->timing = on != 0; }

int grp_set_input_format(svo_group* c, int format) {
    if (converts(format) && !c->ingest_img.d) {
        HIP_TRY(hipSetDevice(c->device));
        if (const int rc = alloc_mirrored_table(c, c->ingest_img, c->ingest_img_host, 2 * (size_t)c->B)) return rc;
    }
    c->input_format = format;
    c->fmt = ingest_format(format);
    return SVO_OK;
}

svo_totals grp_totals(const svo_group* c) {
    svo_totals t = c->totals;
    t.image_sets = c->image_sets;
    return t;
}

const std::vector<svo_launch_shape>& grp_launch_shapes(const svo_group* c) { return c->launch_shapes; }

namespace svo {

void flush_one(Seq& q) {
    if (!q.pending) return;
    q.pending = false;
    float prev_pose[6];
    std::memcpy(prev_pose, q.pose, sizeof(prev_pose));
    std::memcpy(q.pose, q.pending_pose, sizeof(q.pose));
    const double dt = q.pending_ts - q.ts;
    const double inv = 1. / dt;
    float motion[6];
    for (int i = 0; i < 6; i++) motion[i] = (float)((q.pose[i] - prev_pose[i]) * inv);
    const float pv[6] = {0.1f, 0.1f, 0.1f, 0.1f, 0.1f, 0.1f};
    const float mv[6] = {1, 1, 1, 1, 1, 1};
    float filtered[6];
    q.kf.update(q.pose, motion, pv, mv, 0.0, filtered);
    std::memcpy(q.pose, filtered, sizeof(q.pose));
    q.ts = q.pending_ts;
    svo_pose p;
    std::memcpy(&p, q.pose, sizeof(p));
    q.trajectory.push_back(p);
}

void flush_pending(svo_group* c) {
    for (Seq& q : c->seqs) flush_one(q);
}


void end_sequence(svo_group* c, int s) {
    Seq& q = c->seqs[s];
    if (q.frame_id < 0) return;
    flush_one(q);
    FinishedRun f;
    clear(f.info);
    f.info.seq = s; f.info.run = q.run; f.info.frames = q.frame_id + 1; f.info.keyframes = (int)q.kfs.size();
    f.info.last_time_stamp = (float)q.ts;
    std::memcpy(f.info.pose, q.pose, sizeof(f.info.pose));
    f.trajectory = std::move(q.trajectory);
    c->finished.push_back(std::move(f));
    for (KfHost& k : q.kfs) {
        release_set(q, k.set);
        c->kf_slabs.push_back(reinterpret_cast<uint8_t*>(k.kps.kps3d));
    }
    release_set(q, q.cur_set);
    release_set(q, q.prev_set);
    q.kfs.clear();
    q.kfs_retired = 0;
    q.trajectory.clear();
    q.cur = 0; q.n_host = 0; q.frame_id = -1; q.ts = 0; q.run++;
    std::memset(q.pose, 0, sizeof(q.pose));
    q.kf.init();
    clear(q.stats);
}

void trim_keyframes(svo_group* c, Seq& q, int below) {
    const int to = std::min(below, q.kfs_retired);
    if (to <= q.kfs.first()) return;
    for (int id = q.kfs.first(); id < to; id++) {
        KfHost& k = q.kfs[(size_t)id];
        release_set(q, k.set);
        c->kf_slabs.push_back(reinterpret_cast<uint8_t*>(k.kps.kps3d));
    }
    q.kfs.drop_below(to);
}

}

int grp_trim_keyframes(svo_group* c, const int* seqs, const int* below, int n) {
    if (c->failed)
        return svo_set_error(SVO_ERR_INVALID, "svo_submit_trim_keyframes: an earlier frame of this ctx failed; create a new ctx");
    for (int i = 0; i < n; i++) trim_keyframes(c, c->seqs[seqs[i]], below[i]);
    return SVO_OK;
}

void grp_set_keyframe_window(svo_group* c, int keep) { c->kf_window = keep; }

svo_keyframe_range grp_keyframe_range(const svo_group* c, int seq) {
    const Seq& q = c->seqs[seq];
    return svo_keyframe_range{q.kfs.first(), q.kfs_retired, (int)q.kfs.size(), c->max_kf};
}

int grp_restart_sequences(svo_group* c, const int* seqs, int n) {
// ... 38 lines not shown
```

### stereo-svo-slam_amd/csrc/svo_group.hpp

```cpp
#pragma once

#include <cstdint>
#include <memory>
#include <vector>

#include "../../include/svo_hip.h"

namespace svo { struct RemapMap; }
struct svo_group;
struct GroupDelete { void operator()(svo_group* g) const; };
using Group = std::unique_ptr<svo_group, GroupDelete>;

int grp_create(const svo_camera_settings* cam, int width, int height, int n_sequences, int device, Group* out);
int grp_new_images(svo_group* g, const uint8_t* const* left, const uint8_t* const* right, int stride,
                   const float* time_stamps, int mem);
int grp_restart_sequences(svo_group* g, const int* seqs, int n);
int grp_trim_keyframes(svo_group* g, const int* seqs, const int* below, int n);
void grp_set_keyframe_window(svo_group* g, int keep);
svo_keyframe_range grp_keyframe_range(const svo_group* g, int seq);
struct RigBinding {
    int rig;
    svo_camera_settings cam;
    const uint8_t* maps[2];
};
int grp_assign_rigs(svo_group* g, const int* seqs, const RigBinding* b, int n);
int grp_export(svo_group* g, int what, int mem, const int* seqs, const int* seg, int n, int seq0, int64_t base,
               const svo_export_dst* dst);
int grp_export_map(svo_group* g, int mem, const int* seqs, const int* seg, const svo_map_region* regions, int n, int seq0,
                   const svo_map_filter* filter, const svo_map_dst* dst);
int grp_export_views(svo_group* g, int what, int mem, const int* seqs, const int* seg, int n, int seq0,
                     const svo_view_style* style, const svo_view_dst* dst);
int grp_check_view_style(const svo_group* g, const svo_view_style* style);
int64_t grp_view_bytes(const svo_group* g, const svo_view_style* style);
int grp_export_scenes(svo_group* g, int mem, const int* seqs, const int* seg, int n, int seq0, const svo_scene_style* style,
                      const svo_scene_camera* cameras, const svo_scene_dst* dst);
int64_t grp_scene_bytes(const svo_scene_style* style);
struct ArJob {
    svo_ar_style style{};
    struct Mesh { size_t v0, t0, c0; int n_vertices, n_triangles; bool has_rgb; };
    std::vector<Mesh> meshes;
    std::vector<float> vertices;
    std::vector<int32_t> triangles;
    std::vector<uint32_t> rgb;
    std::vector<svo_ar_instance> instances;
};
int grp_export_ar(svo_group* g, int mem, const int* seqs, const int* seg, const int* inst0, const int* inst1, int n, int seq0,
                  const ArJob* job, const svo_ar_dst* dst);
int64_t grp_ar_bytes(const svo_group* g, const svo_ar_style* style);
int grp_export_disparity(svo_group* g, int what, int mem, const int* seqs, const int* seg, int n, int seq0,
                         const svo_disparity_style* style, const svo_disparity_dst* dst);
int grp_check_disparity_style(const svo_group* g, const svo_disparity_style* style);
int64_t grp_disparity_bytes(const svo_group* g, const svo_disparity_style* style);
int grp_export_cloud(svo_group* g, int what, int mem, const int* seqs, const int* seg, int n, int seq0, const svo_cloud_style* style,
                     const svo_cloud_dst* dst);
int grp_check_cloud_style(const svo_group* g, const svo_cloud_style* style);
int64_t grp_cloud_points(const svo_group* g, const svo_cloud_style* style);
void grp_map_size(const svo_group* g, int seq, int from_keyframe, int* keyframes, int64_t* points_bound, int* from = nullptr);
struct SnapshotLoad {
    int seq;
    std::vector<uint8_t> host;
    const void* data;
};
int grp_check_snapshot(const svo_group* g, const svo_camera_settings* slot_cam, const svo_snapshot* snap,
                       std::vector<uint8_t>* host_copy);
int grp_save(svo_group* g, const int* seqs, int n, const svo_snapshot* snaps, int mem);
int grp_load(svo_group* g, const SnapshotLoad* loads, int n, int mem);
int grp_snapshot_size(svo_group* g, int seq, int64_t* host_bytes, int64_t* data_bytes);
int grp_pose_updates(svo_group* g, const int* seqs, const int* counts, int n, const svo_pose_sample* samples,
                     float* const* filtered);
int grp_capacity(const svo_group* g);
void grp_drop_finished_runs(svo_group* g, int seq);
svo_memory grp_memory(const svo_group* g);
void grp_set_exact_pinv(svo_group* g, int on);
void grp_set_rectification(svo_group* g, const svo::RemapMap* maps);
int grp_set_input_format(svo_group* g, int format);
void grp_enable_timing(svo_group* g, int on);
svo_totals grp_totals(const svo_group* g);
const std::vector<svo_launch_shape>& grp_launch_shapes(const svo_group* g);
```

### stereo-svo-slam_amd/csrc/svo_group_state.hpp

```cpp
#pragma once

#include <hip/hip_runtime.h>

#include <algorithm>
#include <cmath>
#include <cstddef>
#include <cstdint>
#include <cstring>
#include <memory>
#include <vector>

#include "svo_group.hpp"
#include "svo_host.hpp"
#include "svo_tracker.hpp"
namespace svo {

struct PoseFilter {
    static constexpr int N = 12;
    float statePre[N], statePost[N];
    float A[N * N], Hm[N * N], Q[N * N], R[N * N];
    float errorCovPre[N * N], errorCovPost[N * N], gain[N * N];

    static void identity(float* m, float v) {
        std::memset(m, 0, sizeof(float) * N * N);
// ... 72 lines not shown
        float z[N];
        for (int i = 0; i < 6; i++) { z[i] = pose[i]; z[6 + i] = speed[i]; }
        correct(z);
        for (int i = 0; i < 6; i++) filtered[i] = statePost[i];
    }
};

struct ImageSet {
    uint8_t* base = nullptr;
    ImgView left[SVO_MAX_PYRAMID_LEVELS];
    ImgView right;
    ImgView lk[SVO_LK_LEVELS];
    ImgView own_left0, own_right;
    int refs = 0;
};

struct SetLayout {
    ImageSet views;
    size_t left[SVO_MAX_PYRAMID_LEVELS], right, lk[SVO_LK_LEVELS];
    size_t bytes;
};

struct FrameResult {
    float pose_sia[6];
    float pose_refined[6];
    float sia_cost, reproj_cost;
    int inside, overflow, kf_n, old_count;
    int min_kf;
    unsigned live_kf[2];
    svo_gn_trace sia_trace[SVO_MAX_PYRAMID_LEVELS];
    svo_gn_trace reproj_trace;
};

struct KfHost {
    ImageSet* set;
    float pose[6];
    int n;
    KpsDev kps;
};

class KfList {
  public:
    int first() const { return first_; }
    size_t size() const { return (size_t)first_ + v_.size(); }
    int resident() const { return (int)v_.size(); }
    bool empty() const { return v_.empty(); }
    KfHost& operator[](size_t id) { return v_[id - (size_t)first_]; }
    const KfHost& operator[](size_t id) const { return v_[id - (size_t)first_]; }
    KfHost& back() { return v_.back(); }
    const KfHost& back() const { return v_.back(); }
    void push_back(const KfHost& k) { v_.push_back(k); }
    std::vector<KfHost>::iterator begin() { return v_.begin(); }
    std::vector<KfHost>::iterator end() { return v_.end(); }
    std::vector<KfHost>::const_iterator begin() const { return v_.begin(); }
    std::vector<KfHost>::const_iterator end() const { return v_.end(); }
    void drop_below(int id) {
        v_.erase(v_.begin(), v_.begin() + (id - first_));
        first_ = id;
    }
    void clear(int first = 0) { v_.clear(); first_ = first; }
  private:
    std::vector<KfHost> v_;
    int first_ = 0;
};

struct Seq {
    KpsDev kps[2];
    int cur = 0;
    int* d_n = nullptr;
    svo_kp2d* tracked = nullptr;
    float* klt_err = nullptr;
    uint8_t* klt_status = nullptr;
    float* disparity = nullptr;
    float* sia_rec = nullptr;
    float* sia_kpws = nullptr;
    PoseMats* sia_mats = nullptr;
    uint8_t* tmpl_base = nullptr;
    uint8_t* tmpl_valid = nullptr;
    KfDev* d_kfs = nullptr;
    KfList kfs;
    int kfs_retired = 0;
    DetCell* det = nullptr; int* n_det = nullptr;
    DetCell* sel = nullptr; int* sel_level = nullptr; int* sel_cell = nullptr; int* occupied = nullptr;
    uint32_t* color_lcg = nullptr;
    std::vector<std::unique_ptr<ImageSet>> sets;
    std::vector<ImageSet*> free_sets;
    ImageSet* cur_set = nullptr;
    ImageSet* prev_set = nullptr;
    int rig = 0;
    svo_camera_settings cam{};
    const uint8_t* rig_maps[2] = {nullptr, nullptr};
    PoseFilter kf;
    int frame_id = -1;
    int run = 0;
    double ts = 0;
    float pose[6] = {0, 0, 0, 0, 0, 0};
    std::vector<svo_pose> trajectory;
    svo_frame_stats stats;
    int n_host = 0;
    bool pending = false;
    float pending_pose[6] = {0, 0, 0, 0, 0, 0};
    double pending_ts = 0;
};

struct FinishedRun {
    svo_run_info info;
    std::vector<svo_pose> trajectory;
};

template <typename T>
struct ArgArray {
    using type = T;
    T* h = nullptr;
    T* d = nullptr;
};

struct ArgBlocks {
    ArgArray<PyrArgs> pyr;
    ArgArray<CompactArgs> compact;
    ArgArray<SiaArgs> sia;
    ArgArray<KltArgs> klt;
    ArgArray<ReprojArgs> reproj;
    ArgArray<SsdArgs> ssd;
    ArgArray<FilterArgs> filter;
    ArgArray<float[8]> guess;
    ArgArray<RemapChunk> remap_chunk;
    ArgArray<DetectArgs> detect;
    ArgArray<MergeArgs> merge;
    ArgArray<KfInitArgs> kf_init;
    ArgArray<int> enable;
    ArgArray<KfDev> kf_record;
    template <typename F> void frame_arrays(F f) { f(pyr); f(compact); f(sia); f(klt); f(reproj); f(ssd); f(filter); f(guess); }
    template <typename F> void rig_arrays(F f) { f(remap_chunk); }
    template <typename F> void keyframe_arrays(F f) { f(detect); f(merge); f(kf_init); f(enable); f(kf_record); }
    PinnedPtr<uint8_t> host;
    uint8_t* dev = nullptr;
    size_t frame_bytes = 0, frame_rig_bytes = 0, bytes = 0;
};

}

struct svo_group {
    svo::Stream stream;
    int device, B, width, height, cap, rec_cap, max_kf, n_lk, det_levels, max_cells, merge_cells;
    svo_camera_settings cam;
    std::vector<svo::DevPtr<void>> dev_mem;
    std::vector<svo::Seq> seqs;
    svo::ArgBlocks args;
    svo::PinnedPtr<uint8_t> readback_host;
    svo::FrameResult* d_res = nullptr; svo::FrameResult* h_res = nullptr;
    int* h_n = nullptr;
    int* d_n_all = nullptr;
    int* d_inside = nullptr; int* h_inside = nullptr;
    size_t readback_bytes = 0;
    uint8_t* d_stage_in = nullptr; size_t stage_frame_bytes = 0;
    const svo::RemapMap* rect = nullptr;
    svo::ArgArray<svo::RemapImg> remap_img;
    svo::PinnedPtr<svo::RemapImg> remap_img_host;
    int input_format = SVO_INPUT_GRAY_PAIR;
    const svo::IngestFormat* fmt = nullptr;
    svo::ArgArray<svo::IngestImg> ingest_img;
    svo::PinnedPtr<svo::IngestImg> ingest_img_host;
    uint8_t* d_raw_gray = nullptr; size_t raw_plane_bytes = 0;
    uint8_t* d_export = nullptr;
    uint8_t* d_snap = nullptr; size_t snap_bytes = 0;
    int* d_map_counts = nullptr; size_t map_counts = 0;
    svo::PinnedPtr<int> map_counts_host;
    svo_map_point* d_map_points = nullptr; size_t map_points = 0;
    uint8_t* d_view = nullptr; size_t view_bytes = 0;
    uint8_t* d_scene_in = nullptr; size_t scene_in_bytes = 0;
    svo::PinnedPtr<uint8_t> scene_in_host;
    uint8_t* d_scene = nullptr; size_t scene_bytes = 0;
    uint8_t* d_ar_in = nullptr; size_t ar_in_bytes = 0;
    svo::PinnedPtr<uint8_t> ar_in_host;
    uint8_t* d_ar_rec = nullptr; size_t ar_rec_bytes = 0;
    uint8_t* d_ar = nullptr; size_t ar_bytes = 0;
    uint8_t* d_dense = nullptr; size_t dense_bytes = 0;
    uint8_t* d_cloud = nullptr; size_t cloud_bytes = 0;
    svo::PinnedPtr<int> cloud_counts_host; size_t cloud_counts_cap = 0;
    uint8_t* d_pose = nullptr; size_t pose_up_bytes = 0, pose_down_bytes = 0;
    svo::PinnedPtr<uint8_t> pose_host;
    bool timing = false;
    bool failed = false;
    int exact_pinv = 1;
    svo::Event ev[10];
    svo::SetLayout set_layout;
    std::vector<uint8_t*> kf_slabs;
    int kf_slab_count = 0;
    size_t device_bytes = 0;
    std::vector<svo::FinishedRun> finished;
    std::vector<uint8_t*> set_slabs;
    int tmpl_kf = 0, tmpl_cap = 0;
    size_t tmpl_block_bytes = 0, tmpl_valid_bytes = 0;
    svo_totals totals;
    std::vector<svo_launch_shape> launch_shapes;
    bool retire_kf_images = true;
    int kf_window = -1;
    int image_sets = 0;
    double host_ms[8] = {0, 0, 0, 0, 0, 0, 0, 0};
    long host_steps = 0;
};

namespace svo {

template <typename T>
T& clear(T& x) {
    std::memset(&x, 0, sizeof(x));
    return x;
}

template <typename T>
int dev_alloc(svo_group* c, T** p, size_t count, bool zero = true) {
    const size_t bytes = sizeof(T) * std::max<size_t>(count, 1);
    DevPtr<void> q;
    HIP_TRY(dev_malloc(q, bytes));
    if (zero) {
        HIP_TRY(hipMemsetAsync(q.get(), 0, bytes, nullptr));
        HIP_TRY(hipStreamSynchronize(nullptr));
    }
    *p = static_cast<T*>(q.get());
    c->dev_mem.push_back(std::move(q));
    c->device_bytes += bytes;
    return SVO_OK;
}

inline bool converts(int format) { return format != SVO_INPUT_GRAY_PAIR && format != SVO_INPUT_SBS_GRAY; }

constexpr int MAX_KEYFRAMES = 4096;

template <typename Tile, typename Launch>
TileTable<Tile, Launch> group_tile_table(svo_group* c, const char* env, Launch run) {
    return {reinterpret_cast<Tile*>(c->args.host.get()), reinterpret_cast<Tile*>(c->args.dev),
            table_tiles(env, c->args.bytes / sizeof(Tile)), c->stream.get(), run};
}

size_t align_up(size_t v, size_t a);
// ... 14 lines not shown
```

### stereo-svo-slam_amd/csrc/svo_group_step.hip

```cpp
#include <hip/hip_runtime.h>

#include <algorithm>
#include <chrono>
#include <cstring>
#include <vector>

#include "svo_group_state.hpp"

using namespace svo;

namespace {

struct Step {
    const uint8_t* const* left;
    const uint8_t* const* right;
    int stride, mem;
    const float* time_stamps;
    std::vector<int> act;
    std::vector<int> trk;
    std::vector<int> start;
    std::vector<int> need;
    int pyr_stream = -1;
    struct Remap { const uint8_t* map[2]; RemapImg left, right; };
    std::vector<Remap> remap;
// ... 246 lines not shown
            launch_ingest(c->ingest_img.d + i0, std::min(32768, 2 * M - i0), c->width, c->height, st);
            HIP_TRY(hipGetLastError());
        }
    }
    if (const int R = (int)s.remap.size()) {
        HIP_TRY(hipMemcpyAsync(c->remap_img.d, c->remap_img.h, sizeof(RemapImg) * 2 * R, hipMemcpyHostToDevice, st));
        if (s.remap_shared) {
            RemapLaunch ra;
            for (int side = 0; side < 2; side++)
                ra.map[side] = remap_map_view(const_cast<uint8_t*>(s.remap[0].map[side]), c->width, c->height);
            ra.img = c->remap_img.d; ra.n = R;
            launch_remap(ra, 2, st);
        } else {
            RemapMultiLaunch ra;
            clear(ra);
            ra.chunks = a.remap_chunk.d; ra.img = c->remap_img.d; ra.n = R;
            launch_remap_multi(ra, c->width, c->height, s.remap_chunks, s.remap_single, 2, st);
        }
        HIP_TRY(hipGetLastError());
    }
    launch_pyr_fused(a.pyr.d, M, c->width, c->height, s.copy_right, std::max(s.pyr_stream, 0), st);
    HIP_TRY(hipGetLastError());
    HIP_TRY(mark(c, 1));
    if (T == 0) {
        for (int i = 2; i <= 7; i++) HIP_TRY(mark(c, i));
        return SVO_OK;
    }
    launch_compact(a.compact.d, T, c->cap, st);
    HIP_TRY(hipGetLastError());
    HIP_TRY(mark(c, 2));
    int grid_n = 1;
    for (int seq : s.trk) grid_n = std::max(grid_n, c->seqs[seq].n_host);
    grid_n = std::min(grid_n, c->cap);
    const LaunchStatus sia_launch =
        launch_sia(a.sia.d, T, c->cam, c->width, c->height, grid_n, c->rec_cap, c->exact_pinv, st);
    HIP_TRY(sia_launch.err);
    if (!sia_launch.shape.fits)
        return svo_set_error(SVO_ERR_CAPACITY, "sparse alignment: %d keypoints exceed the workspaces", grid_n);
    count_launch(c, SVO_KERNEL_SIA_GN, sia_launch.shape);
    HIP_TRY(hipGetLastError());
    HIP_TRY(mark(c, 3));
    launch_klt(a.klt.d, T, grid_n, c->cam.window_size_opt_flow, st);
    HIP_TRY(hipGetLastError());
    HIP_TRY(mark(c, 4));
    const LaunchStatus reproj_launch = launch_reproj(a.reproj.d, T, grid_n, st);
    HIP_TRY(reproj_launch.err);
    if (!reproj_launch.shape.fits)
        return svo_set_error(SVO_ERR_CAPACITY, "reprojection GN: %d keypoints do not fit LDS", grid_n);
    count_launch(c, SVO_KERNEL_REPROJ_GN, reproj_launch.shape);
    HIP_TRY(hipGetLastError());
    HIP_TRY(mark(c, 5));
    launch_ssd(a.ssd.d, T, grid_n, c->cam.window_size_depth_calculator, c->cam.search_y, st);
    HIP_TRY(hipGetLastError());
    HIP_TRY(mark(c, 6));
    launch_filter(a.filter.d, T, grid_n, st);
    HIP_TRY(hipGetLastError());
    HIP_TRY(mark(c, 7));
    HIP_TRY(hipMemcpyAsync(c->h_inside, c->d_inside, sizeof(int) * c->B, hipMemcpyDeviceToHost, st));
    return SVO_OK;
}

int new_keyframe_storage(svo_group* c, Seq& q, int s, int id) {
    if (id - q.kfs.first() >= c->max_kf)
        return svo_set_error(SVO_ERR_CAPACITY, "more than %d resident keyframes (svo_trim_keyframes makes room)", c->max_kf);
    KfHost k{};
    if (const int rc = take_kf_slab(c, &k.kps)) return rc;
    k.set = q.cur_set;
    q.cur_set->refs++;
    q.kfs.push_back(k);
    fill_kf_record(c, q, id, k, c->args.kf_record.h[s]);
    return SVO_OK;
}

int pack_keyframe_args(svo_group* c, int slot, int s, bool first_frame) {
    ArgBlocks& a = c->args;
    Seq& q = c->seqs[s];
    FrameResult* dr = c->d_res + s;
    const int id = (int)q.kfs.size();
    const int rc = new_keyframe_storage(c, q, s, id);
    if (rc) return rc;
    CompactArgs& ca = pack_compact(c, q, slot, 1);
    ca.width = c->width; ca.height = c->height;
    ca.zero = q.n_det; ca.zero_count = SVO_MAX_PYRAMID_LEVELS;
    if (first_frame) {
        ca.start = 1;
        ca.zero_res = reinterpret_cast<int*>(dr); ca.zero_res_count = (int)(sizeof(FrameResult) / sizeof(int));
    }
    DetectArgs& da = clear(a.detect.h[slot]);
    for (int l = 0; l < c->cam.max_pyramid_levels; l++) da.level[l] = q.cur_set->left[l];
    da.n_levels = c->det_levels; da.grid_w = c->cam.grid_width; da.grid_h = c->cam.grid_height;
    da.out = q.det; da.n_out = q.n_det; da.max_cells = c->max_cells;
    MergeArgs& ma = clear(a.merge.h[slot]);
    ma.cam = q.cam; ma.width = c->width; ma.height = c->height;
    ma.det = q.det; ma.n_det = q.n_det; ma.n_levels = c->det_levels; ma.max_cells = c->max_cells;
    ma.kps = q.kps[q.cur]; ma.cap = c->cap;
    ma.sel = q.sel; ma.sel_level = q.sel_level; ma.sel_cell = q.sel_cell; ma.occupied = q.occupied;
    ma.old_count = &dr->old_count; ma.overflow = &dr->overflow;
    pack_ssd(c, q, slot, 0, &dr->old_count);
    KfInitArgs& ia = clear(a.kf_init.h[slot]);
    ia.cam = q.cam; ia.kps = q.kps[q.cur]; ia.old_count = &dr->old_count;
    ia.disparity = q.disparity; ia.frame_pose = dr->pose_refined;
    ia.first_frame = first_frame ? 1 : 0; ia.new_kf_id = id; ia.kfs = q.d_kfs; ia.kf_mask = c->max_kf - 1;
    ia.color_lcg = q.color_lcg; ia.n_out = &dr->kf_n;
    ia.record = a.kf_record.h[s];
    ia.tmpl_valid_bytes = (int)c->tmpl_valid_bytes;
    ia.evict_id = (c->tmpl_kf > 0 && id - c->tmpl_kf >= q.kfs.first()) ? id - c->tmpl_kf : -1;
    return SVO_OK;
}

int enqueue_keyframes(svo_group* c, const Step& s) {
    const ArgBlocks& a = c->args;
    hipStream_t st = c->stream.get();
    int m = 0;
    for (int seq = 0; seq < c->B; seq++) {
        if (!s.need[seq]) continue;
        const int rc = pack_keyframe_args(c, m++, seq, s.start[seq] != 0);
        if (rc) return rc;
    }
    if (m == 0) return SVO_OK;
    HIP_TRY(hipMemcpyAsync(a.dev, a.host.get(), a.bytes, hipMemcpyHostToDevice, st));
    launch_compact(a.compact.d, m, c->cap, st);
    HIP_TRY(hipGetLastError());
    if (c->det_levels > 0) {
        launch_detect(a.detect.d, m, c->max_cells, c->det_levels, c->cam.grid_width, c->cam.grid_height, st);
        HIP_TRY(hipGetLastError());
    }
    launch_select_merge(a.merge.d, m, c->max_cells, st);
    HIP_TRY(hipGetLastError());
    launch_ssd(a.ssd.d, m, c->cap, c->cam.window_size_depth_calculator, c->cam.search_y, st);
    HIP_TRY(hipGetLastError());
    launch_kf_init(a.kf_init.d, m, st);
    HIP_TRY(hipGetLastError());
    return SVO_OK;
}

int decide_keyframes(svo_group* c, Step& s) {
    const int max_keypoints = (c->width / c->cam.grid_width) * (c->height / c->cam.grid_height);
    bool any = false;
    for (int seq : s.act) {
        s.need[seq] = s.start[seq] || (double)c->h_inside[seq] < 0.66 * max_keypoints ? 1 : 0;
        any = any || s.need[seq];
    }
    return any ? enqueue_keyframes(c, s) : SVO_OK;
}

int read_stage_times(svo_group* c, Step& s) {
    HIP_TRY(mark(c, 8));
    if (!c->timing) return SVO_OK;
    HIP_TRY(hipEventSynchronize(c->ev[8].get()));
    for (int i = 0; i < 8; i++) (void)hipEventElapsedTime(&s.stage_ms[i], c->ev[i].get(), c->ev[i + 1].get());
    return SVO_OK;
}

void retire_keyframe_images(svo_group* c, const Step& s) {
    for (int seq : s.trk) {
        Seq& q = c->seqs[seq];
        const FrameResult& r = c->h_res[seq];
        const int newest = (int)q.kfs.size() - 1;
        for (; q.kfs_retired < std::min(r.min_kf, newest); q.kfs_retired++) release_set(q, q.kfs[q.kfs_retired].set);
        for (int i = 0; i < 64 && r.min_kf < newest && r.min_kf + i < newest; i++) {
            KfHost& old = q.kfs[r.min_kf + i];
            if (old.set && !((r.live_kf[i >> 5] >> (i & 31)) & 1u)) release_set(q, old.set);
        }
    }
}

int book_frame(svo_group* c, Step& s) {
    int overflow_seq = -1;
    for (int seq : s.act) {
        Seq& q = c->seqs[seq];
        const FrameResult& r = c->h_res[seq];
        const double ts = (double)s.time_stamps[seq];
        const bool first = s.start[seq] != 0;
        q.frame_id++;
        if (first) {
            std::memset(q.pose, 0, sizeof(q.pose));
            q.ts = ts;
            q.trajectory.push_back(svo_pose{});
        } else {
            q.pending = true;
            std::memcpy(q.pending_pose, r.pose_refined, sizeof(q.pending_pose));
            q.pending_ts = ts;
        }
        if (s.need[seq]) {
            KfHost& k = q.kfs.back();
            k.n = r.kf_n;
            if (first) std::memset(k.pose, 0, sizeof(k.pose));
            else std::memcpy(k.pose, r.pose_refined, sizeof(k.pose));
        }
        q.n_host = c->h_n[2 * seq + q.cur];
        svo_frame_stats& st = clear(q.stats);
        st.frame_id = q.frame_id; st.is_keyframe = s.need[seq]; st.n_keypoints = q.n_host;
        st.n_keyframes = (int)q.kfs.size(); st.inside_count = first ? 0 : c->h_inside[seq]; st.overflow = r.overflow;
        std::memcpy(st.pose_sia, r.pose_sia, sizeof(st.pose_sia));
        std::memcpy(st.pose_refined, r.pose_refined, sizeof(st.pose_refined));
        st.sia_cost = r.sia_cost; st.reproj_cost = r.reproj_cost; st.sia_ms = s.stage_ms[2];
        std::memcpy(st.stage_ms, s.stage_ms, sizeof(s.stage_ms));
        std::memcpy(st.sia_trace, r.sia_trace, sizeof(st.sia_trace));
        st.reproj_trace = r.reproj_trace;
        c->totals.frames++;
        c->totals.keyframes += s.need[seq];
        c->totals.keypoints += q.n_host;
        if (!first)
            for (int l = 0; l < SVO_MAX_PYRAMID_LEVELS; l++) {
                c->totals.gn_gradient_calls += r.sia_trace[l].n_gradient;
                c->totals.gn_cost_calls += r.sia_trace[l].n_cost;
            }
        if (r.overflow && overflow_seq < 0) overflow_seq = seq;
    }
    lap(c, s, 6);
    c->host_steps++;
    c->totals.launches++;
// ... 54 lines not shown
```

### stereo-svo-slam_amd/csrc/svo_handle.hpp

```cpp
#pragma once

#include <cstdint>
#include <vector>

#include "svo_host.hpp"
#include "svo_kernels.hpp"
#include "svo_tracker.hpp"

struct svo_workspace {
    svo::DevPtr<uint8_t> ptr;
    size_t bytes = 0;
    int reserve(size_t need, hipStream_t stream) {
        if (need <= bytes) return SVO_OK;
        HIP_TRY(hipStreamSynchronize(stream));
        ptr.reset();
        bytes = 0;
        HIP_TRY(svo::dev_malloc(ptr, need));
        bytes = need;
        return SVO_OK;
    }
};

struct svo_handle {
    int device;
    hipStream_t stream = nullptr;
    int max_kps;
    svo::DevPtr<uint8_t> ring;
    size_t ring_cap = 1 << 20, ring_off = 0;
    svo::DevPtr<float> sia_kpws;
    svo::DevPtr<float> sia_rec;
    int rec_cap;
    int exact_pinv = 1;
    svo_workspace remap_ws;
    svo_workspace rigcam_ws;
    svo_workspace ingest_ws;
    svo_workspace export_ws;
    svo_workspace copy_ws;
    svo_workspace map_ws;
    svo_workspace view_ws;
    svo_workspace scene_ws;
    svo_workspace ar_ws;
    svo_workspace dense_ws;
    svo_workspace cloud_ws;
};

#define CHECK_H(h)                                                   \
    do {                                                             \
        if (!(h)) return svo_set_error(SVO_ERR_INVALID, "null handle");       \
        HIP_TRY(hipSetDevice((h)->device));                          \
    } while (0)

template <typename T>
int stage(svo_handle* h, const T* host, size_t count, T** dev) {
    const size_t bytes = (sizeof(T) * count + 255) & ~(size_t)255;
    if (bytes > h->ring_cap) return svo_set_error(SVO_ERR_CAPACITY, "argument blocks do not fit the ring");
    if (h->ring_off + bytes > h->ring_cap) {
        HIP_TRY(hipStreamSynchronize(h->stream));
        h->ring_off = 0;
    }
    T* d = reinterpret_cast<T*>(h->ring.get() + h->ring_off);
    h->ring_off += bytes;
    HIP_TRY(hipMemcpyAsync(d, host, sizeof(T) * count, hipMemcpyHostToDevice, h->stream));
    *dev = d;
    return SVO_OK;
}
template <typename T>
int stage(svo_handle* h, const T& host, T** dev) { return stage(h, &host, 1, dev); }
template <typename T>
int stage(svo_handle* h, const std::vector<T>& host, T** dev) { return stage(h, host.data(), host.size(), dev); }
inline int stage_n(svo_handle* h, int n, int** d_n) { return stage(h, &n, 1, d_n); }

inline int finish_launch(svo_handle* h) {
    const hipError_t launched = hipGetLastError();
    HIP_TRY(hipStreamSynchronize(h->stream));
    HIP_TRY(launched);
    return SVO_OK;
}

enum : unsigned {
    KP_KPS2D = 1 << 0, KP_KPS3D = 1 << 1, KP_FLAGS = 1 << 2, KP_KF_ID = 1 << 3, KP_KP_INDEX = 1 << 4, KP_OUTL = 1 << 5,
    KP_INL = 1 << 6, KP_KFX = 1 << 7, KP_KFP = 1 << 8, KP_SCORE = 1 << 9, KP_LEVEL_TYPE = 1 << 10, KP_COLOR = 1 << 11,
    KP_ALL = (1 << 12) - 1,
    KP_MAP = KP_KPS3D | KP_FLAGS | KP_KF_ID | KP_INL | KP_COLOR,
    KP_VIEW = KP_KPS2D | KP_FLAGS | KP_LEVEL_TYPE | KP_COLOR,
};

inline bool take_planes(const svo_keypoints& k, unsigned planes, bool non_empty, svo::KpsDev& d) {
    bool ok = true;
    auto take = [&](unsigned bit, auto*& dst, auto* src) {
        if (!(planes & bit)) return;
        dst = src;
        ok = ok && (src || !non_empty) && !((uintptr_t)src & 3);
    };
    d = svo::KpsDev{};
    take(KP_KPS2D, d.kps2d, k.kps2d);
    take(KP_KPS3D, d.kps3d, k.kps3d);
    take(KP_FLAGS, d.flags, k.flags);
    take(KP_KF_ID, d.kf_id, k.keyframe_id);
    take(KP_KP_INDEX, d.kp_index, k.keypoint_index);
    take(KP_OUTL, d.outl, k.outlier_count);
    take(KP_INL, d.inl, k.inlier_count);
    take(KP_KFX, d.kfx, k.kf_inv_depth);
    take(KP_KFP, d.kfP, k.kf_variance);
    take(KP_SCORE, d.score, k.score);
    take(KP_LEVEL_TYPE, d.level_type, k.level_type);
    take(KP_COLOR, d.color, k.color);
    return ok;
}
```

### stereo-svo-slam_amd/csrc/svo_tracker.hpp

```cpp
#pragma once

#include <vector>

#include "../../include/svo_hip.h"
#include "svo_kernels.hpp"

namespace svo {

struct KpsDev {
    svo_kp2d* kps2d;
    svo_kp3d* kps3d;
    uint32_t* flags;
    int* kf_id;
    int* kp_index;
    int* outl;
    int* inl;
    float* kfx;
    float* kfP;
    float* score;
    int* level_type;
    uint32_t* color;
    int* n;
};

inline void fill_filter_table_args(FilterArgs& fa, const svo_camera_settings& cam, const KpsDev& k, const float* frame_pose,
                                   const float* disparity, KfDev* kfs, int kf_mask, int width, int height,
                                   int* inside_count) {
    fa.cam = cam; fa.n_ptr = k.n; fa.frame_pose = frame_pose;
    fa.kps2d = k.kps2d; fa.kps3d = k.kps3d; fa.flags = k.flags;
    fa.outlier_count = k.outl; fa.inlier_count = k.inl; fa.kf_inv_depth = k.kfx;
    fa.kf_variance = k.kfP; fa.disparity = disparity;
    fa.kfs = kfs; fa.kf_mask = kf_mask; fa.kf_id = k.kf_id; fa.kp_index = k.kp_index;
    fa.do_outlier_check = 1; fa.do_update = 1; fa.do_flags = 1; fa.do_reproject = 1;
    fa.width = width; fa.height = height; fa.inside_count = inside_count;
}

struct CompactArgs {
    KpsDev src, dst;
    int mode;
    int width, height;
    const int* enable;
    int* zero;
    int zero_count;
    int start;
    int* zero_res;
    int zero_res_count;
    int* min_kf;
};
void launch_compact(const CompactArgs* d_args, int batch, int cap, hipStream_t stream);
int compact_pick_threads(int cap);

struct DetCell {
    float x, y, score;
    int type;
};

struct DetectArgs {
    ImgView level[SVO_MAX_PYRAMID_LEVELS];
    int n_levels;
    int grid_w, grid_h;
    DetCell* out;
    int* n_out;
    int max_cells;
    const int* enable;
};
void launch_detect(const DetectArgs* d_args, int batch, int max_cells, int n_levels, int grid_w, int grid_h, hipStream_t stream);
struct DetectShape { int cell_w, cell_h, list; };
DetectShape detect_pick_shape(int grid_w, int grid_h);

struct MergeArgs {
    svo_camera_settings cam;
    int width, height;
    const DetCell* det;
    const int* n_det;
    int n_levels, max_cells;
    KpsDev kps;
    int cap;
    DetCell* sel;
    int* sel_level;
    int* sel_cell;
    int* occupied;
    int* old_count;
    int* overflow;
    const int* enable;
};
void launch_select_merge(const MergeArgs* d_args, int batch, int max_cells, hipStream_t stream);
int select_merge_pick_threads(int max_cells);

constexpr uint32_t SVO_COLOR_LCG_SEED = 12345u;

struct KfInitArgs {
    svo_camera_settings cam;
    KpsDev kps;
    const int* old_count;
    const float* disparity;
    const float* frame_pose;
    int first_frame;
    int new_kf_id;
    int kf_mask;
    KfDev* kfs;
    uint32_t* color_lcg;
    int* n_out;
    const int* enable;
    KfDev record;
    int tmpl_valid_bytes;
    int evict_id;
};
void launch_kf_init(const KfInitArgs* d_args, int batch, hipStream_t stream);
inline size_t kf_tmpl_valid_bytes(int tmpl_cap) { return ((size_t)tmpl_cap * SVO_LK_LEVELS + 255) / 256 * 256; }

constexpr int EXPORT_TILE = 256;
constexpr int EXPORT_PLANES = 10;
struct ExportTile {
    const uint32_t* kps2d;
    const uint32_t* kps3d;
    const uint32_t* plane[EXPORT_PLANES];
    int64_t first;
    int count, pad_;
};
ExportTile export_tile(const KpsDev& k, int start, int count, int64_t first);
void launch_export(const ExportTile* d_tiles, int n_tiles, svo_kp2d* kps2d, svo_kp3d* kps3d, svo_kp_info* info,
                   hipStream_t stream);

constexpr int MAP_TILE = 256;
struct MapTile {
    const uint32_t* kps3d;
    const uint32_t* flags;
    const int* kf_id;
    const int* inl;
    const uint32_t* color;
    int64_t first;
    int count;
    int own_id;
    int index;
    int region_tile;
    int set_tile;
    int set;
};
void map_tiles(const KpsDev& k, int n, int own_id, int set, int64_t first, int region_tile, std::vector<MapTile>& out);
void launch_map(const MapTile* d_tiles, int n_tiles, const svo_map_filter& filter, svo_map_point* points,
                int* tile_counts, int* set_counts, hipStream_t stream);

constexpr int COPY_TILE_BYTES = 32768;
struct CopyTile {
    const uint8_t* src;
    uint8_t* dst;
    int64_t src_pitch, dst_pitch;
    int row_bytes, rows;
};
void cut_copy_tiles(const void* src, void* dst, int64_t row_bytes, int64_t rows, int64_t src_pitch, int64_t dst_pitch,
                    std::vector<CopyTile>& out);
void launch_copy_tiles(const CopyTile* d_tiles, int n_tiles, hipStream_t stream);

constexpr int VIEW_TILE_W = 64, VIEW_TILE_H = 16;
struct ViewTile {
    const uint8_t* src;
    uint8_t* dst;
    const svo_kp2d* kps2d;
    const uint32_t* flags;
    const int* level_type;
    const uint32_t* color;
    int src_stride, w, h;
    int x0, y0;
    int n;
// ... 136 lines not shown
```

### stereo-svo-slam_amd/stereo_svo_slam_amd/hip_lib.py

```python
import ctypes as C
import os

import numpy as np
import torch

_HERE = os.path.dirname(os.path.abspath(__file__))
CSRC = os.path.normpath(os.path.join(_HERE, "..", "csrc"))
LIB_PATH = os.environ.get("SVO_HIP_LIB", os.path.join(CSRC, "libsvo_hip.so"))
_LIB = None

SYMBOLS = (
    "svo_last_error", "svo_version", "svo_handle_create", "svo_handle_destroy",
    "svo_handle_set_stream", "svo_handle_synchronize", "svo_build_pyramid",
    "svo_build_lk_pyramid", "svo_sparse_align", "svo_klt_track", "svo_reproj_gn",
    "svo_ssd_disparity", "svo_depth_filter_update",
    "svo_ctx_create", "svo_ctx_destroy", "svo_new_images", "svo_submit_images", "svo_wait",
    "svo_ctx_get_groups", "svo_new_image", "svo_get_pose",
    "svo_get_frame_keypoints", "svo_get_keyframe_count", "svo_get_keyframe",
    "svo_get_trajectory", "svo_update_pose", "svo_get_frame_stats", "svo_ctx_enable_timing",
    "svo_get_totals", "svo_handle_set_exact_pinv", "svo_ctx_set_exact_pinv",
    "svo_handle_set_fast_solver", "svo_ctx_set_fast_solver",
    "svo_device_malloc", "svo_device_free", "svo_copy_to_device", "svo_copy_to_host",
    "svo_copy_image_to_device", "svo_project_keypoints",
    "svo_ctx_get_launch_shapes", "svo_pick_launch_shapes", "svo_pick_sia_lds_bytes", "svo_pinv6_check",
    "svo_solve6_check", "svo_remap_linear", "svo_ctx_set_rectification",
    "svo_detect_keypoints", "svo_detect_shape",
    "svo_ctx_restart_sequences", "svo_get_finished_runs", "svo_get_finished_run",
    "svo_drop_finished_runs", "svo_ctx_get_memory",
    "svo_input_format_info", "svo_convert_frames", "svo_ctx_set_input_format",
    "svo_export_capacity", "svo_submit_export", "svo_export", "svo_pack_keypoints",
    "svo_snapshot_size", "svo_submit_save", "svo_save_sequences", "svo_submit_load", "svo_load_sequences",
    "svo_snapshot_info", "svo_copy_segments",
    "svo_reproj_gn_batch", "svo_filter_update_batch", "svo_sparse_align_batch",
    "svo_submit_pose_updates", "svo_update_poses", "svo_pose_filter_batch",
    "svo_map_size", "svo_submit_export_map", "svo_export_map", "svo_pack_map_points",
    "svo_view_size", "svo_submit_export_views", "svo_export_views", "svo_render_views",
    "svo_disparity_size", "svo_submit_export_disparity", "svo_export_disparity", "svo_dense_disparity",
    "svo_cloud_size", "svo_submit_export_cloud", "svo_export_cloud", "svo_cloud_points",
    "svo_scene_size", "svo_scene_look_at", "svo_scene_frustum", "svo_submit_export_scenes", "svo_export_scenes",
    "svo_render_scene",
    "svo_ar_size", "svo_ar_camera_of_pose", "svo_submit_export_ar", "svo_export_ar", "svo_render_ar",
    "svo_remap_linear_multi", "svo_ctx_add_rigs", "svo_ctx_remove_rigs", "svo_ctx_assign_rigs", "svo_ctx_get_slot_rig",
    "svo_ctx_get_rigs",
    "svo_klt_track_batch", "svo_klt_cache_layout",
    "svo_rectify_inverse", "svo_build_rectify_maps", "svo_ctx_add_rigs_calibrated", "svo_ctx_set_calibration",
    "svo_submit_trim_keyframes", "svo_trim_keyframes", "svo_ctx_set_keyframe_window", "svo_get_keyframe_range",
    "svo_keyframe_launch_info", "svo_compact_batch", "svo_keyframe_merge_batch", "svo_keyframe_init_batch",
    "svo_keyframe_record_layout", "svo_ssd_disparity_batch",
    "svo_sparse_align_batch_mats", "svo_pose_mats_layout", "svo_filter_update_table_batch",
    "svo_sia_records_check",
)

INPUT_GRAY_PAIR, INPUT_BGR_PAIR, INPUT_RGB_PAIR, INPUT_SBS_GRAY, INPUT_SBS_BGR, INPUT_SBS_RGB, INPUT_CH3_ECON = range(7)
INPUT_FORMATS = ("gray_pair", "bgr_pair", "rgb_pair", "sbs_gray", "sbs_bgr", "sbs_rgb", "ch3_econ")
INGEST_COPY, INGEST_GRAY = 0, 1
EXPORT_FRAMES, EXPORT_LAST_KEYFRAMES = 0, 1
EXPORT_WHAT = ("frames", "last_keyframes")
MEM_HOST, MEM_DEVICE = 0, 1


class SvoError(RuntimeError):
    pass


class CameraSettings(C.Structure):
    _fields_ = [(n, C.c_float) for n in
                ("baseline", "fx", "fy", "cx", "cy", "k1", "k2", "k3", "p1", "p2")] + \
               [(n, C.c_int32) for n in
                ("grid_height", "grid_width", "search_x", "search_y",
                 "window_size_pose_estimator", "window_size_opt_flow",
                 "window_size_depth_calculator", "max_pyramid_levels",
                 "min_pyramid_level_pose_estimation")]

    @classmethod
    def from_dict(cls, d):
        cam = cls()
        for name, _ in cls._fields_:
            setattr(cam, name, d[name])
        return cam


RIG_FLOATS = ("baseline", "fx", "fy", "cx", "cy", "k1", "k2", "k3", "p1", "p2")


class Rig(C.Structure):
    _fields_ = [(n, C.c_float) for n in RIG_FLOATS] + \
               [(n, C.c_void_p) for n in ("left_map_x", "left_map_y", "right_map_x", "right_map_y")] + \
               [("mem", C.c_int32), ("_reserved", C.c_int32)]

    @classmethod
    def from_dict(cls, d):
        get = d.__getitem__ if isinstance(d, dict) else lambda n: getattr(d, n)
        return cls(**{n: get(n) for n in RIG_FLOATS})


assert C.sizeof(Rig) == 80


class CameraCalibration(C.Structure):
    _fields_ = [("K", C.c_double * 9), ("D", C.c_double * 8), ("R", C.c_double * 9), ("P", C.c_double * 9)]

    @classmethod
    def from_mats(cls, K, D, R, P):
        K, P = np.asarray(K, np.float64), np.asarray(P, np.float64)
        D = np.asarray(D, np.float64).ravel()
        R = np.eye(3) if R is None else np.asarray(R, np.float64)
        if K.shape != (3, 3) or R.shape != (3, 3) or P.shape not in ((3, 3), (3, 4)):
            raise ValueError(f"K, R are 3x3 and P is 3x3 or 3x4, not {K.shape}, {R.shape}, {P.shape}")
        if D.size not in (4, 5, 8):
            raise ValueError(f"D has 4, 5 or 8 coefficients, not {D.size}")
        cal = cls()
        cal.K[:] = K.ravel().tolist()
        cal.D[:] = D.tolist() + [0.0] * (8 - D.size)
        cal.R[:] = R.ravel().tolist()
        cal.P[:] = P[:, :3].ravel().tolist()
        return cal


assert C.sizeof(CameraCalibration) == 280


class Image(C.Structure):
    _fields_ = [("data", C.c_void_p), ("width", C.c_int32), ("height", C.c_int32),
                ("stride", C.c_int32)]


class KltKeyframe(C.Structure):
    _fields_ = [("lk", Image * 3), ("n_lk", C.c_int32), ("n_kps", C.c_int32), ("kps2d", C.c_void_p),
                ("tmpl", C.c_void_p), ("tmpl_valid", C.c_void_p), ("tmpl_bytes", C.c_int64),
                ("tmpl_valid_bytes", C.c_int64), ("tmpl_cap", C.c_int32), ("tmpl_win", C.c_int32)]


class KltSequence(C.Structure):
    _fields_ = [("kfs", C.POINTER(KltKeyframe)), ("n_kfs", C.c_int32), ("n_cur", C.c_int32), ("cur", Image * 3),
                ("n", C.c_void_p), ("kf_id", C.c_void_p), ("kp_index", C.c_void_p), ("kps3d", C.c_void_p),
                ("pose", C.c_void_p), ("cam", CameraSettings)] + \
               [(n, C.c_void_p) for n in ("tracked", "status", "err", "proj_out", "ref_out")]


assert (C.sizeof(KltKeyframe), C.sizeof(KltSequence)) == (128, 248)


KPS_PLANES = ("kps2d", "kps3d", "flags", "kf_id", "kp_index", "outlier_count", "inlier_count", "kf_inv_depth",
              "kf_variance", "score", "level_type", "color", "n")


class KpsPlanes(C.Structure):
    _fields_ = [(name, C.c_void_p) for name in KPS_PLANES]


class CompactSequence(C.Structure):
    _fields_ = [("src", KpsPlanes), ("dst", KpsPlanes), ("mode", C.c_int32), ("width", C.c_int32), ("height", C.c_int32),
                ("start", C.c_int32), ("enable", C.c_void_p), ("zero", C.c_void_p), ("zero_res", C.c_void_p),
                ("min_kf", C.c_void_p), ("zero_count", C.c_int32), ("zero_res_count", C.c_int32)]


class MergeSequence(C.Structure):
    _fields_ = [("cam", CameraSettings), ("width", C.c_int32), ("height", C.c_int32), ("det", C.c_void_p),
                ("n_det", C.c_void_p), ("kps", KpsPlanes), ("sel", C.c_void_p), ("sel_level", C.c_void_p),
                ("sel_cell", C.c_void_p), ("occupied", C.c_void_p), ("old_count", C.c_void_p), ("overflow", C.c_void_p),
                ("enable", C.c_void_p), ("occupied_count", C.c_int32), ("pad_", C.c_int32)]


class KfInitSequence(C.Structure):
    _fields_ = [("cam", CameraSettings), ("first_frame", C.c_int32), ("new_kf_id", C.c_int32), ("kf_mask", C.c_int32),
                ("evict_id", C.c_int32), ("kps", KpsPlanes), ("record", KpsPlanes), ("old_count", C.c_void_p),
                ("disparity", C.c_void_p), ("frame_pose", C.c_void_p), ("kfs", C.c_void_p), ("kfs_bytes", C.c_int64),
                ("color_lcg", C.c_void_p), ("n_out", C.c_void_p), ("enable", C.c_void_p), ("tmpl", C.c_void_p),
                ("tmpl_valid", C.c_void_p), ("tmpl_valid_bytes", C.c_int32), ("tmpl_cap", C.c_int32),
                ("tmpl_win", C.c_int32), ("pad_", C.c_int32)]


class SsdSequence(C.Structure):
    _fields_ = [("left", Image), ("right", Image), ("n", C.c_void_p), ("kps2d", C.c_void_p), ("disparity", C.c_void_p),
                ("win", C.c_int32), ("search_x", C.c_int32), ("search_y", C.c_int32), ("clamp_half", C.c_int32),
                ("first", C.c_int32), ("cap", C.c_int32), ("first_ptr", C.c_void_p), ("enable", C.c_void_p)]


class FilterKeyframe(C.Structure):
    _fields_ = [("pose", C.c_float * 6)] + \
               [(n, C.c_void_p) for n in ("kps2d", "kps3d", "flags", "outlier_count", "inlier_count")] + \
               [("n", C.c_int32), ("pad_", C.c_int32)]


class FilterTableSequence(C.Structure):
    _fields_ = [("cam", CameraSettings), ("kps", KpsPlanes), ("frame_pose", C.c_void_p), ("disparity", C.c_void_p),
                ("kfs", C.POINTER(FilterKeyframe)), ("records", C.c_void_p), ("records_bytes", C.c_int64),
                ("table", C.c_int32), ("kf_mask", C.c_int32), ("width", C.c_int32), ("height", C.c_int32),
                ("inside_count", C.c_void_p)]


assert (C.sizeof(KpsPlanes), C.sizeof(CompactSequence), C.sizeof(MergeSequence), C.sizeof(KfInitSequence),
        C.sizeof(SsdSequence), C.sizeof(FilterKeyframe), C.sizeof(FilterTableSequence)) == (104, 264, 272, 400, 112, 72, 248)


def _addr(x):
    if x is None:
        return None
    if isinstance(x, int):
        return C.c_void_p(x)
    assert x.is_cuda
    return C.c_void_p(x.data_ptr())


def _fill(struct, d, skip=()):
    for name, typ in struct._fields_:
        if name in skip or name not in d or d[name] is None:
            continue
        v = d[name]
        if typ is C.c_void_p:
            setattr(struct, name, _addr(v))
        elif typ is KpsPlanes:
            _fill(getattr(struct, name), v)
        elif typ in (C.c_int32, C.c_int64):
            setattr(struct, name, int(v))
        else:
            setattr(struct, name, v)


class InputSide(C.Structure):
    _fields_ = [("buffer", C.c_int32), ("start_column", C.c_int32), ("op", C.c_int32), ("channel", C.c_int32),
                ("weight", C.c_int32 * 3)]


class InputLayout(C.Structure):
    _fields_ = [("buffers", C.c_int32), ("channels", C.c_int32), ("min_row_pixels", C.c_int32),
                ("left", InputSide), ("right", InputSide)]


GN_TRACE_DTYPE = np.dtype([("level", "<i4"), ("n_gradient", "<i4"), ("n_cost", "<i4"),
                           ("n_accepted", "<i4"), ("exit_small", "<i4"),
                           ("initial_cost", "<f4"), ("final_cost", "<f4"), ("pose", "<f4", (6,))])
assert GN_TRACE_DTYPE.itemsize == 52


DET_CELL_DTYPE = np.dtype([("x", "<f4"), ("y", "<f4"), ("score", "<f4"), ("type", "<i4")])
assert DET_CELL_DTYPE.itemsize == 16


EXPORT_SEGMENT_DTYPE = np.dtype([("seq", "<i4"), ("run", "<i4"), ("frame_id", "<i4"), ("keyframe_id", "<i4"),
                                 ("is_keyframe", "<i4"), ("n", "<i4"), ("first", "<i8"), ("pose", "<f4", (6,)),
                                 ("time_stamp", "<f4"), ("_pad", "<i4")])
assert EXPORT_SEGMENT_DTYPE.itemsize == 64

# ... 866 lines not shown
        return out, sweeps

    def reproj_gn(self, kps2d, kps3d, flags, cam, pose_in, tracked=None, err=None):
        dev = kps2d.device
        n = kps2d.shape[0]
        pose_out = torch.zeros(6, dtype=torch.float32, device=dev)
        cost = torch.zeros(1, dtype=torch.float32, device=dev)
        trace = torch.zeros(GN_TRACE_DTYPE.itemsize, dtype=torch.uint8, device=dev)
        _check(lib().svo_reproj_gn(self._h, _ptr(kps2d), _ptr(kps3d), _ptr(flags), n, C.byref(cam),
                                   _ptr(tracked), _ptr(err), _ptr(pose_in), _ptr(pose_out),
                                   _ptr(cost), _ptr(trace)))
        return pose_out, cost, trace

    def reproj_gn_batch(self, n, n_bound, kps2d, kps3d, flags, cam, pose_in, tracked=None, err=None, zero_out=None):
        batch, stride = kps2d.shape[0], kps2d.shape[1]
        dev = kps2d.device
        pose_out = torch.zeros((batch, 6), dtype=torch.float32, device=dev)
        cost = torch.zeros(batch, dtype=torch.float32, device=dev)
        trace = torch.zeros((batch, GN_TRACE_DTYPE.itemsize), dtype=torch.uint8, device=dev)
        waves, cap = C.c_int(0), C.c_int(0)
        _check(lib().svo_reproj_gn_batch(self._h, batch, stride, _ptr(n), int(n_bound), _ptr(kps2d), _ptr(kps3d),
                                         _ptr(flags), C.byref(cam), _ptr(tracked), _ptr(err), _ptr(pose_in),
                                         _ptr(pose_out), _ptr(cost), _ptr(trace), _ptr(zero_out), C.byref(waves),
                                         C.byref(cap)))
        return pose_out, cost, trace, waves.value, cap.value

    def ssd_disparity(self, left, right, kps2d, win, search_x, search_y, clamp_half=1):
        n = kps2d.shape[0]
        out = torch.zeros(n, dtype=torch.float32, device=kps2d.device)
        a, b = _img(left), _img(right)
        _check(lib().svo_ssd_disparity(self._h, C.byref(a), C.byref(b), _ptr(kps2d), n, win,
                                       search_x, search_y, clamp_half, _ptr(out)))
        return out

    def depth_filter_update(self, kps2d, kps3d, flags, cam, frame_pose, disparity, ref3d, ref2d,
                            kf_pose, outlier, inlier, kf_x, kf_p, do_outlier_check=1, do_update=1):
        n = kps2d.shape[0]
        _check(lib().svo_depth_filter_update(
            self._h, _ptr(kps2d), _ptr(kps3d), _ptr(flags), n, C.byref(cam), _ptr(frame_pose),
            _ptr(disparity), _ptr(ref3d), _ptr(ref2d), _ptr(kf_pose), _ptr(outlier), _ptr(inlier),
            _ptr(kf_x), _ptr(kf_p), do_outlier_check, do_update))

    def filter_update_batch(self, n, n_bound, kps2d, kps3d, flags, cam, frame_pose, disparity, ref3d, ref2d, kf_pose,
                            outlier, inlier, kf_x, kf_p, do_outlier_check, do_update, do_flags, do_reproject, width,
                            height, inside_count):
        batch, stride = kps2d.shape[0], kps2d.shape[1]
        _check(lib().svo_filter_update_batch(
            self._h, batch, stride, _ptr(n), int(n_bound), _ptr(kps2d), _ptr(kps3d), _ptr(flags), C.byref(cam),
            _ptr(frame_pose), _ptr(disparity), _ptr(ref3d), _ptr(ref2d), _ptr(kf_pose), _ptr(outlier), _ptr(inlier),
            _ptr(kf_x), _ptr(kf_p), int(do_outlier_check), int(do_update), int(do_flags), int(do_reproject),
            int(width), int(height), _ptr(inside_count)))

    def filter_update_table_batch(self, seqs, n_bound, do_outlier_check=1, do_update=1, do_flags=1, do_reproject=1):
        arr = (FilterTableSequence * len(seqs))()
        keep = []
        for a, s in zip(arr, seqs):
            kfs = (FilterKeyframe * max(len(s["kfs"]), 1))()
            keep.append(kfs)
            for k, f in zip(kfs, s["kfs"]):
                _fill(k, f, skip=("pose",))
                k.pose[:] = [float(v) for v in f["pose"]]
            _fill(a, s, skip=("kfs", "table"))
            a.kfs, a.table = kfs, int(s.get("table", len(s["kfs"])))
        _check(lib().svo_filter_update_table_batch(self._h, len(seqs), arr, int(n_bound), int(do_outlier_check),
                                                   int(do_update), int(do_flags), int(do_reproject)))

    def compact_batch(self, seqs, cap):
        arr = (CompactSequence * len(seqs))()
        for a, s in zip(arr, seqs):
            _fill(a, s)
        threads = C.c_int(0)
        _check(lib().svo_compact_batch(self._h, len(seqs), arr, int(cap), C.byref(threads)))
        return threads.value

    def keyframe_merge_batch(self, seqs, n_levels, max_cells, cap):
        arr = (MergeSequence * len(seqs))()
        for a, s in zip(arr, seqs):
            _fill(a, s)
        threads = C.c_int(0)
        _check(lib().svo_keyframe_merge_batch(self._h, len(seqs), arr, int(n_levels), int(max_cells), int(cap),
                                              C.byref(threads)))
        return threads.value

    def keyframe_init_batch(self, seqs, cap):
        arr = (KfInitSequence * len(seqs))()
        for a, s in zip(arr, seqs):
            _fill(a, s)
        _check(lib().svo_keyframe_init_batch(self._h, len(seqs), arr, int(cap)))

    def ssd_disparity_batch(self, seqs, n_bound, win, search_y):
        arr = (SsdSequence * len(seqs))()
        for a, s in zip(arr, seqs):
            _fill(a, s, skip=("left", "right"))
            a.left, a.right = _img(s["left"]), _img(s["right"])
        max_win = C.c_int(0)
        _check(lib().svo_ssd_disparity_batch(self._h, len(seqs), arr, int(n_bound), int(win), int(search_y),
                                             C.byref(max_win)))
        return max_win.value


def detect_to_numpy(cells, counts):
    c = cells.cpu().numpy().view(DET_CELL_DTYPE)[..., 0]
    return [c[l, :k].copy() for l, k in enumerate(counts.cpu().numpy())]


def trace_to_numpy(t):
    return t.cpu().numpy().view(GN_TRACE_DTYPE)
```

### stereo-svo-slam_amd/stereo_svo_slam_amd/stereo_slam.py

```python
import ctypes as C

import numpy as np
import torch

from . import hip_lib
from .hip_lib import POSE_SAMPLE_CHAIN, POSE_SAMPLE_DTYPE, CameraSettings, SvoError, _check, lib

KP_INFO_DTYPE = np.dtype([
    ("score", "<f4"), ("level", "<i4"), ("type", "<i4"), ("keyframe_id", "<i4"),
    ("keypoint_index", "<i4"), ("color", "u1", (3,)), ("ignore_during_refinement", "u1"),
    ("ignore_completely", "u1"), ("ignore_temporary", "u1"), ("_pad", "u1", (2,)),
    ("outlier_count", "<i4"), ("inlier_count", "<i4"), ("kf_inv_depth", "<f4"),
    ("kf_variance", "<f4")], align=False)
assert KP_INFO_DTYPE.itemsize == 44


class GnTrace(C.Structure):
    _fields_ = [("level", C.c_int32), ("n_gradient", C.c_int32), ("n_cost", C.c_int32),
                ("n_accepted", C.c_int32), ("exit_small", C.c_int32),
                ("initial_cost", C.c_float), ("final_cost", C.c_float), ("pose", C.c_float * 6)]


class FrameStats(C.Structure):
    _fields_ = [("frame_id", C.c_int32), ("is_keyframe", C.c_int32), ("n_keypoints", C.c_int32),
# ... 855 lines not shown
                if calibrated:
                    left = (hip_lib.CameraCalibration * n)(*[cals[i][0] for i in idx])
                    right = (hip_lib.CameraCalibration * n)(*[cals[i][1] for i in idx])
                    _check(lib().svo_ctx_add_rigs_calibrated(self._ctx, sub, left, right, n, ids))
                else:
                    _check(lib().svo_ctx_add_rigs(self._ctx, sub, n, ids))
                for k, i in enumerate(idx):
                    out[i] = ids[k]
                added += list(ids[:n])
        except SvoError:
            if added:
                _check(lib().svo_ctx_remove_rigs(self._ctx, (C.c_int * len(added))(*added), len(added)))
            raise
        for i in range(len(rigs)):
            cam = CameraSettings.from_buffer_copy(self.cam)
            for name in hip_lib.RIG_FLOATS:
                setattr(cam, name, getattr(arr[i], name))
            self._rig_settings()[out[i]] = bytes(cam)
        return out

    def _rig_settings(self):
        if getattr(self, "_rig_cams", None) is None:
            self._rig_cams = {0: bytes(self.cam)}
        return self._rig_cams

    def remove_rigs(self, ids):
        ids = [int(i) for i in ([ids] if np.isscalar(ids) else ids)]
        _check(lib().svo_ctx_remove_rigs(self._ctx, (C.c_int * max(len(ids), 1))(*ids), len(ids)))
        for i in ids:
            self._rig_settings().pop(i, None)

    def assign_rigs(self, seqs, rigs):
        seqs, rigs = [int(s) for s in seqs], [int(r) for r in rigs]
        assert len(seqs) == len(rigs)
        n = len(seqs)
        _check(lib().svo_ctx_assign_rigs(self._ctx, (C.c_int * max(n, 1))(*seqs), (C.c_int * max(n, 1))(*rigs), n))

    def slot_rig(self, seq):
        rig, cam = C.c_int(0), CameraSettings()
        _check(lib().svo_ctx_get_slot_rig(self._ctx, seq, C.byref(rig), C.byref(cam)))
        return rig.value, cam

    def rigs(self):
        n, b = C.c_int(0), C.c_int64(0)
        _check(lib().svo_ctx_get_rigs(self._ctx, C.byref(n), C.byref(b)))
        return n.value, b.value

    def find_rig(self, cam, add=False):
        for rid, b in self._rig_settings().items():
            if b == bytes(cam):
                return rid
        return self.add_rigs([cam])[0] if add else None

    def finished_runs(self, seq):
        n = C.c_int(0)
        _check(lib().svo_get_finished_runs(self._ctx, seq, C.byref(n)))
        out = []
        for i in range(n.value):
            info, m = RunInfo(), C.c_int(0)
            _check(lib().svo_get_finished_run(self._ctx, seq, i, C.byref(info), None, 0, C.byref(m)))
            traj = np.zeros((m.value, 6), np.float32)
            _check(lib().svo_get_finished_run(self._ctx, seq, i, None, traj.ctypes.data_as(C.c_void_p), m.value, None))
            out.append((info, traj))
        return out

    def drop_finished_runs(self, seq=-1):
        _check(lib().svo_drop_finished_runs(self._ctx, seq))

    def memory(self):
        m = Memory()
        _check(lib().svo_ctx_get_memory(self._ctx, C.byref(m)))
        return m

    def groups(self):
        n = C.c_int(0)
        _check(lib().svo_ctx_get_groups(self._ctx, C.byref(n)))
        return n.value

    def totals(self):
        t = Totals()
        _check(lib().svo_get_totals(self._ctx, C.byref(t)))
        return t

    def launch_shapes(self):
        n = C.c_int(0)
        _check(lib().svo_ctx_get_launch_shapes(self._ctx, None, 0, C.byref(n)))
        out = (LaunchShape * max(n.value, 1))()
        _check(lib().svo_ctx_get_launch_shapes(self._ctx, out, n.value, C.byref(n)))
        return {_shape_key(e): e.launches for e in out[:n.value]}

    def pose(self, seq=0):
        p = np.zeros(6, np.float32)
        _check(lib().svo_get_pose(self._ctx, seq, p.ctypes.data_as(C.c_void_p)))
        return p

    def stats(self, seq=0):
        st = FrameStats()
        _check(lib().svo_get_frame_stats(self._ctx, seq, C.byref(st)))
        return st

    def get_frame(self, seq=0):
        n = C.c_int(0)
        _check(lib().svo_get_frame_keypoints(self._ctx, seq, None, None, None, 0, C.byref(n)))
        k2 = np.zeros((n.value, 2), np.float32)
        k3 = np.zeros((n.value, 3), np.float32)
        info = np.zeros(n.value, KP_INFO_DTYPE)
        _check(lib().svo_get_frame_keypoints(self._ctx, seq, k2.ctypes.data_as(C.c_void_p),
                                             k3.ctypes.data_as(C.c_void_p),
                                             info.ctypes.data_as(C.c_void_p), n.value, C.byref(n)))
        return Frame(self.pose(seq), k2, k3, info)

    def num_keyframes(self, seq=0):
        n = C.c_int(0)
        _check(lib().svo_get_keyframe_count(self._ctx, seq, C.byref(n)))
        return n.value

    def get_keyframe(self, kid=None, seq=0):
        if kid is None:
            kid = self.num_keyframes(seq) - 1
        n = C.c_int(0)
        pose = np.zeros(6, np.float32)
        _check(lib().svo_get_keyframe(self._ctx, seq, kid, None, None, None,
                                      pose.ctypes.data_as(C.c_void_p), 0, C.byref(n)))
        k2 = np.zeros((n.value, 2), np.float32)
        k3 = np.zeros((n.value, 3), np.float32)
        info = np.zeros(n.value, KP_INFO_DTYPE)
        _check(lib().svo_get_keyframe(self._ctx, seq, kid, k2.ctypes.data_as(C.c_void_p),
                                      k3.ctypes.data_as(C.c_void_p), info.ctypes.data_as(C.c_void_p),
                                      pose.ctypes.data_as(C.c_void_p), n.value, C.byref(n)))
        return Frame(pose, k2, k3, info)

    def get_keyframes(self, seq=0):
        return [self.get_keyframe(i, seq) for i in range(self.keyframe_range(seq).first, self.num_keyframes(seq))]

    def get_trajectory(self, seq=0):
        n = C.c_int(0)
        _check(lib().svo_get_trajectory(self._ctx, seq, None, 0, C.byref(n)))
        out = np.zeros((n.value, 6), np.float32)
        _check(lib().svo_get_trajectory(self._ctx, seq, out.ctypes.data_as(C.c_void_p), n.value,
                                        C.byref(n)))
        return out

    def update_pose(self, pose, speed, pose_variance, speed_variance, dt, seq=0):
        out = np.zeros(6, np.float32)
        arrs = [np.ascontiguousarray(a, np.float32) for a in (pose, speed, pose_variance, speed_variance)]
        _check(lib().svo_update_pose(self._ctx, seq, *[a.ctypes.data_as(C.c_void_p) for a in arrs],
                                     C.c_double(dt), out.ctypes.data_as(C.c_void_p)))
        return out


    IMU_RATE = 104.0

    def submit_pose_updates(self, seqs, samples_per_seq):
        seqs = None if seqs is None else [int(s) for s in seqs]
        n = self.n if seqs is None else len(seqs)
        assert len(samples_per_seq) == n
        per = [np.zeros(0, POSE_SAMPLE_DTYPE) if a is None else np.ascontiguousarray(a, POSE_SAMPLE_DTYPE).reshape(-1)
               for a in samples_per_seq]
        counts = (C.c_int * max(n, 1))(*[len(a) for a in per])
        samples = np.concatenate(per) if per else np.zeros(0, POSE_SAMPLE_DTYPE)
        filtered = np.zeros((len(samples), 6), np.float32)
        seq_arr = None if seqs is None else (C.c_int * max(n, 1))(*seqs)
        _check(lib().svo_submit_pose_updates(self._ctx, seq_arr, counts, n, samples.ctypes.data if len(samples) else None,
                                             filtered.ctypes.data if len(samples) else None))
        return filtered

# ... 104 lines not shown
```

Measured before the change: 294,900.

## Skip keyframe detection cells whose merge cells are all occupied

The compact kernel now builds the merge-cell occupancy map while compacting keypoints. It marks each detection cell as skippable when every merge cell it overlaps is already occupied, and the detect kernel exits early for those cells with a zero result. The merge kernel reuses the precomputed occupancy and caches per-candidate cells in LDS for the rank loop, and the SSD launch bound is capped at max_cells. This trades an extra occupancy check inside compaction and an atomic counter for skipping FAST detection work whose output the merge step would discard anyway.

Result: slower. 271,900 (-7.8%).

```diff
diff --git a/include/svo_hip.h b/include/svo_hip.h
--- a/include/svo_hip.h
+++ b/include/svo_hip.h
@@ -648,6 +648,7 @@
     int32_t image_sets;
 } svo_totals;
 int svo_get_totals(svo_ctx *ctx, svo_totals *out);
+int svo_ctx_get_detect_skipped(svo_ctx *ctx, int64_t *cells);
 int svo_ctx_enable_timing(svo_ctx *ctx, int on);
 int svo_ctx_set_fast_solver(svo_ctx *ctx, int on);
 int svo_ctx_set_exact_pinv(svo_ctx *ctx, int on);
@@ -761,6 +762,13 @@
 } svo_merge_sequence;
 int svo_keyframe_merge_batch(svo_handle *h, int batch, const svo_merge_sequence *seqs, int n_levels, int max_cells,
                              int cap, int *threads);
+typedef struct svo_keyframe_candidates_sequence {
+    svo_compact_sequence compact;
+    svo_merge_sequence merge;
+    svo_image levels[SVO_MAX_PYRAMID_LEVELS];
+} svo_keyframe_candidates_sequence;
+int svo_keyframe_candidates_batch(svo_handle *h, int batch, const svo_keyframe_candidates_sequence *seqs, int n_levels,
+                                  int max_cells, int cap, int skip, uint64_t *skipped);
 typedef struct svo_kf_init_sequence {
     svo_camera_settings cam;
     int32_t first_frame, new_kf_id, kf_mask, evict_id;
diff --git a/stereo-svo-slam_amd/csrc/keyframe.hip b/stereo-svo-slam_amd/csrc/keyframe.hip
--- a/stereo-svo-slam_amd/csrc/keyframe.hip
+++ b/stereo-svo-slam_amd/csrc/keyframe.hip
@@ -1,6 +1,7 @@
 #include "svo_kernels.hpp"
 #include "svo_tracker.hpp"
 #include <cstdlib>
+#include <cstring>
 
 namespace svo {
 
@@ -40,6 +41,38 @@
     G(d.color)[di] = G(s.color)[si];
 }
 
+__device__ inline int merge_cell_of(float x, float y, int mcw, int mch, int ncx, int ncy) {
+    if (!(x > 0 && y > 0)) return -1;
+    const int xi = (int)floorf(x) / mcw, yi = (int)floorf(y) / mch;
+    if (xi >= ncx || yi >= ncy) return -1;
+    const int l = xi * mcw, t = yi * mch;
+    return (x > l && x < l + mcw && y > t && y < t + mch) ? xi * ncy + yi : -1;
+}
+
+__device__ inline bool detect_index_skippable(const CompactArgs& a, int cell) {
+    const DetectGrid& g = a.det;
+    const int mncx = (a.width + a.merge_cw - 1) / a.merge_cw, mncy = (a.height + a.merge_ch - 1) / a.merge_ch;
+    for (int l = 0; l < g.n_levels; l++) {
+        const int gw = g.grid_w >> l, gh = g.grid_h >> l;
+        if (gw <= 0 || gh <= 0 || gw > g.max_cell_w || gh > g.max_cell_h) {
+            if (l == 0) return false;
+            continue;
+        }
+        const int ncx = g.w[l] / gw, ncy = max(g.h[l] / gh, 1);
+        if (ncx <= 0 || cell >= ncx * ncy) {
+            if (l == 0) return false;
+            continue;
+        }
+        const int left = (cell % ncx) * gw, top = (cell / ncx) * gh;
+        const int xa = (left << l) / a.merge_cw, xb = min(((left + gw - 1) << l) / a.merge_cw, mncx - 1);
+        const int ya = (top << l) / a.merge_ch, yb = min(((top + gh - 1) << l) / a.merge_ch, mncy - 1);
+        for (int xi = xa; xi <= xb; xi++)
+            for (int yi = ya; yi <= yb; yi++)
+                if (!G(a.occupied)[xi * mncy + yi]) return false;
+    }
+    return true;
+}
+
 __global__ __launch_bounds__(1024) void compact_kernel(const CompactArgs* __restrict__ args) {
     const CompactArgs& a = args[blockIdx.x];
     if (a.enable && !*G(a.enable)) return;
@@ -51,6 +84,9 @@
     const int n = a.start ? 0 : *G(a.src.n);
     const int per = (n + (int)blockDim.x - 1) / (int)blockDim.x;
     const int i0 = tid * per, i1 = min(n, i0 + per);
+    const bool occ = a.occupied && a.mode == 1 && a.merge_cw > 0 && a.merge_ch > 0;
+    const int occ_ncx = occ ? (a.width + a.merge_cw - 1) / a.merge_cw : 0, occ_ncy = occ ? (a.height + a.merge_ch - 1) / a.merge_ch : 0;
+    for (int c = tid; c < occ_ncx * occ_ncy; c += blockDim.x) G(a.occupied)[c] = 0;
     int cnt = 0;
     for (int i = i0; i < i1; i++) {
         const uint32_t f = G(a.src.flags)[i];
@@ -80,11 +116,24 @@
         if (keep) {
             copy_kp(a.dst, pos++, a.src, i);
             min_kf = min(min_kf, G(a.src.kf_id)[i]);
+            if (occ) {
+                const svo_kp2d k = G(a.src.kps2d)[i];
+                const int mc = merge_cell_of(k.x, k.y, a.merge_cw, a.merge_ch, occ_ncx, occ_ncy);
+                if (mc >= 0) G(a.occupied)[mc] = 1;
+            }
         }
     }
     if (tid == 0) {
         *G(a.dst.n) = total;
         if (a.start) *G(a.src.n) = 0;
+    }
+    if (occ && a.skip) {
+        __syncthreads();
+        for (int j = tid; j < a.skip_count; j += blockDim.x) {
+            const int s = detect_index_skippable(a, j) ? 1 : 0;
+            G(a.skip)[j] = s;
+            if (s && a.skipped) atomicAdd(G(a.skipped), 1ull);
+        }
     }
     if (a.min_kf) {
         if (min_kf != INT_MAX) atomicMin(&s_min_kf, min_kf);
@@ -187,6 +236,15 @@
     const int cxi = cell % ncx, cyi = cell / ncx;
     const int left = cxi * gw, top = cyi * gh;
     const int tid = threadIdx.x;
+    if (a.skip && G(a.skip)[cell]) {
+        if (tid == 0) {
+            DetCell o;
+            o.x = 0.f; o.y = 0.f; o.score = 0.f; o.type = SVO_KP_FAST;
+            G(a.out)[(size_t)level * a.max_cells + cell] = o;
+            if (cell == 0) G(a.n_out)[level] = ncx * ncy;
+        }
+        return;
+    }
 
     __shared__ __attribute__((aligned(16))) uint8_t s_t[DET_TH * DET_TW];
     __shared__ uint8_t s_raw[DET_RH * DET_RW];
@@ -309,12 +367,24 @@
     return grid_w <= DET_SMALL.cell_w && grid_h <= DET_SMALL.cell_h ? DET_SMALL : DET_LARGE;
 }
 
+DetectGrid detect_grid(const DetectArgs& da) {
+    DetectGrid g;
+    memset(&g, 0, sizeof(g));
+    const DetectShape s = detect_pick_shape(da.grid_w, da.grid_h);
+    g.n_levels = da.n_levels; g.grid_w = da.grid_w; g.grid_h = da.grid_h;
+    g.max_cell_w = s.cell_w; g.max_cell_h = s.cell_h;
+    for (int l = 0; l < da.n_levels && l < SVO_MAX_PYRAMID_LEVELS; l++) { g.w[l] = da.level[l].w; g.h[l] = da.level[l].h; }
+    return g;
+}
+
 void launch_detect(const DetectArgs* d_args, int batch, int max_cells, int n_levels, int grid_w, int grid_h, hipStream_t stream) {
     if (detect_pick_shape(grid_w, grid_h).cell_w == DET_SMALL.cell_w)
         hipLaunchKernelGGL((kf_detect_kernel<DET_SMALL.cell_w, DET_SMALL.cell_h, DET_SMALL.list>), dim3(max_cells, n_levels, batch), dim3(256), 0, stream, d_args);
     else
         hipLaunchKernelGGL((kf_detect_kernel<DET_LARGE.cell_w, DET_LARGE.cell_h, DET_LARGE.list>), dim3(max_cells, n_levels, batch), dim3(256), 0, stream, d_args);
 }
+
+constexpr int MERGE_LDS_CELLS = 2048;
 
 __global__ __launch_bounds__(1024) void kf_select_merge_kernel(const MergeArgs* __restrict__ args) {
     const MergeArgs& a = args[blockIdx.x];
@@ -325,6 +395,8 @@
     const int mcw = a.cam.grid_height, mch = a.cam.grid_width;
     const int ncx = (a.width + mcw - 1) / mcw, ncy = (a.height + mch - 1) / mch;
     const int ncells = ncx * ncy;
+    __shared__ int s_cell[MERGE_LDS_CELLS];
+    const bool lds = nsel <= MERGE_LDS_CELLS;
 
     for (int j = tid; j < nsel; j += nthr) {
         DetCell s = G(a.det)[j];
@@ -341,39 +413,42 @@
         }
         G(a.sel)[j] = s;
         G(a.sel_level)[j] = lvl;
-        G(a.sel_cell)[j] = -1;
-    }
-    for (int c = tid; c < ncells; c += nthr) G(a.occupied)[c] = 0;
-    __syncthreads();
-    for (int i = tid; i < n_old; i += nthr) {
-        const svo_kp2d k = G(a.kps.kps2d)[i];
-        if (!(k.x > 0 && k.y > 0)) continue;
-        const int xi = (int)floorf(k.x) / mcw, yi = (int)floorf(k.y) / mch;
-        if (xi >= ncx || yi >= ncy) continue;
-        const int l = xi * mcw, t = yi * mch;
-        if (k.x > l && k.x < l + mcw && k.y > t && k.y < t + mch) G(a.occupied)[xi * ncy + yi] = 1;
+    }
+    if (!a.occupied_ready) {
+        for (int c = tid; c < ncells; c += nthr) G(a.occupied)[c] = 0;
+        __syncthreads();
+        for (int i = tid; i < n_old; i += nthr) {
+            const svo_kp2d k = G(a.kps.kps2d)[i];
+            const int mc = merge_cell_of(k.x, k.y, mcw, mch, ncx, ncy);
+            if (mc >= 0) G(a.occupied)[mc] = 1;
+        }
     }
     __syncthreads();
     for (int j = tid; j < nsel; j += nthr) {
         const DetCell s = G(a.sel)[j];
-        if (!(s.x > 0 && s.y > 0)) continue;
-        const int xi = (int)floorf(s.x) / mcw, yi = (int)floorf(s.y) / mch;
-        if (xi >= ncx || yi >= ncy) continue;
-        const int l = xi * mcw, t = yi * mch;
-        if (s.x > l && s.x < l + mcw && s.y > t && s.y < t + mch && !G(a.occupied)[xi * ncy + yi])
-            G(a.sel_cell)[j] = xi * ncy + yi;
+        int mc = merge_cell_of(s.x, s.y, mcw, mch, ncx, ncy);
+        if (mc >= 0 && G(a.occupied)[mc]) mc = -1;
+        G(a.sel_cell)[j] = mc;
+        if (lds) s_cell[j] = mc;
     }
     __syncthreads();
     __shared__ int s_cnt;
     if (tid == 0) s_cnt = 0;
     __syncthreads();
     for (int j = tid; j < nsel; j += nthr) {
-        const int cj = G(a.sel_cell)[j];
+        const int cj = lds ? s_cell[j] : G(a.sel_cell)[j];
         if (cj < 0) continue;
         int pos = 0;
-        for (int q = 0; q < nsel; q++) {
-            const int cq = G(a.sel_cell)[q];
-            pos += (cq >= 0 && (cq < cj || (cq == cj && q < j))) ? 1 : 0;
+        if (lds) {
+            for (int q = 0; q < nsel; q++) {
+                const int cq = s_cell[q];
+                pos += (cq >= 0 && (cq < cj || (cq == cj && q < j))) ? 1 : 0;
+            }
+        } else {
+            for (int q = 0; q < nsel; q++) {
+                const int cq = G(a.sel_cell)[q];
+                pos += (cq >= 0 && (cq < cj || (cq == cj && q < j))) ? 1 : 0;
+            }
         }
         atomicAdd(&s_cnt, 1);
         const int di = n_old + pos;
diff --git a/stereo-svo-slam_amd/csrc/svo_capi.hip b/stereo-svo-slam_amd/csrc/svo_capi.hip
--- a/stereo-svo-slam_amd/csrc/svo_capi.hip
+++ b/stereo-svo-slam_amd/csrc/svo_capi.hip
@@ -312,7 +312,7 @@
     return SVO_OK;
 }
 
-static int check_detect_levels(const char* who, int n_levels, int grid_width, int grid_height) {
+int check_detect_levels(const char* who, int n_levels, int grid_width, int grid_height) {
     if (n_levels < 1 || n_levels > SVO_MAX_PYRAMID_LEVELS)
         return svo_set_error(SVO_ERR_INVALID, "%s: n_levels must be 1..%d", who, SVO_MAX_PYRAMID_LEVELS);
     if (grid_width < 4 || grid_height < 4 || grid_width > 96 || grid_height > 64)
@@ -321,7 +321,7 @@
         return svo_set_error(SVO_ERR_INVALID, "%s: the cell of level %d is empty", who, n_levels - 1);
     return SVO_OK;
 }
-static int detect_level_cells(const char* who, int l, int width, int height, int grid_width, int grid_height, int* cells) {
+int detect_level_cells(const char* who, int l, int width, int height, int grid_width, int grid_height, int* cells) {
     const int gw = grid_width >> l, gh = grid_height >> l;
     if (width < 1 || height < gh)
         return svo_set_error(SVO_ERR_INVALID, "%s: level %d (%d x %d) is lower than its cell (%d x %d)", who, l, width, height, gw, gh);
diff --git a/stereo-svo-slam_amd/csrc/svo_capi_check.hip b/stereo-svo-slam_amd/csrc/svo_capi_check.hip
--- a/stereo-svo-slam_amd/csrc/svo_capi_check.hip
+++ b/stereo-svo-slam_amd/csrc/svo_capi_check.hip
@@ -614,42 +614,75 @@
     return SVO_OK;
 }
 
+static int fill_compact_args(const char* who, int b, const svo_compact_sequence& s, int cap, CompactArgs& ca) {
+    if (planes_missing(s.src, true) || planes_missing(s.dst, true) || (s.mode != 0 && s.mode != 1) ||
+        (s.start != 0 && s.start != 1) || s.zero_count < 0 || s.zero_res_count < 0 || (s.zero_count > 0 && !s.zero) ||
+        (s.zero_res_count > 0 && !s.zero_res))
+        return svo_set_error(SVO_ERR_INVALID, "%s: sequence %d: bad arguments", who, b);
+    if (s.min_kf && s.mode != 0)
+        return svo_set_error(SVO_ERR_INVALID, "%s: sequence %d: min_kf is defined for mode 0 only", who, b);
+    if (!s.start) {
+        int32_t n = 0;
+        if (const int rc = read_i32(s.src.n, 1, &n)) return rc;
+        if (n < 0 || n > cap)
+            return svo_set_error(SVO_ERR_INVALID, "%s: sequence %d: n = %d is outside 0..cap = %d", who, b, n, cap);
+    }
+    memset(&ca, 0, sizeof(ca));
+    ca.src = kps_dev(s.src); ca.dst = kps_dev(s.dst); ca.mode = s.mode;
+    ca.width = s.width; ca.height = s.height;
+    ca.enable = s.enable;
+    ca.zero = s.zero; ca.zero_count = s.zero_count;
+    ca.start = s.start;
+    ca.zero_res = s.zero_res; ca.zero_res_count = s.zero_res_count;
+    ca.min_kf = s.min_kf;
+    return SVO_OK;
+}
+
 extern "C" int svo_compact_batch(svo_handle* h, int batch, const svo_compact_sequence* seqs, int cap, int* threads) {
     CHECK_H(h);
     if (bad_batch(batch, seqs) || cap < 1)
         return svo_set_error(SVO_ERR_INVALID, "svo_compact_batch: need 1 <= batch <= 4096, seqs and cap >= 1");
     HIP_TRY(hipStreamSynchronize(h->stream));
     std::vector<CompactArgs> blocks((size_t)batch);
-    for (int b = 0; b < batch; b++) {
-        const svo_compact_sequence& s = seqs[b];
-        if (planes_missing(s.src, true) || planes_missing(s.dst, true) || (s.mode != 0 && s.mode != 1) ||
-            (s.start != 0 && s.start != 1) || s.zero_count < 0 || s.zero_res_count < 0 || (s.zero_count > 0 && !s.zero) ||
-            (s.zero_res_count > 0 && !s.zero_res))
-            return svo_set_error(SVO_ERR_INVALID, "svo_compact_batch: sequence %d: bad arguments", b);
-        if (s.min_kf && s.mode != 0)
-            return svo_set_error(SVO_ERR_INVALID, "svo_compact_batch: sequence %d: min_kf is defined for mode 0 only", b);
-        if (!s.start) {
-            int32_t n = 0;
-            if (const int rc = read_i32(s.src.n, 1, &n)) return rc;
-            if (n < 0 || n > cap)
-                return svo_set_error(SVO_ERR_INVALID, "svo_compact_batch: sequence %d: n = %d is outside 0..cap = %d", b, n, cap);
-        }
-        CompactArgs& ca = blocks[(size_t)b];
-        memset(&ca, 0, sizeof(ca));
-        ca.src = kps_dev(s.src); ca.dst = kps_dev(s.dst); ca.mode = s.mode;
-        ca.width = s.width; ca.height = s.height;
-        ca.enable = s.enable;
-        ca.zero = s.zero; ca.zero_count = s.zero_count;
-        ca.start = s.start;
-        ca.zero_res = s.zero_res; ca.zero_res_count = s.zero_res_count;
-        ca.min_kf = s.min_kf;
-    }
+    for (int b = 0; b < batch; b++)
+        if (const int rc = fill_compact_args("svo_compact_batch", b, seqs[b], cap, blocks[(size_t)b])) return rc;
     CompactArgs* d;
     const int rc = stage(h, blocks, &d);
     if (rc) return rc;
     if (threads) *threads = compact_pick_threads(cap);
     launch_compact(d, batch, cap, h->stream);
     return finish_launch(h);
+}
+
+static int fill_merge_args(const char* who, int b, const svo_merge_sequence& s, int n_levels, int max_cells, int cap, bool counts,
+                           MergeArgs& ma) {
+    if (planes_missing(s.kps, true) || !s.det || !s.n_det || !s.sel || !s.sel_level || !s.sel_cell || !s.occupied ||
+        !s.old_count || !s.overflow || s.width < 1 || s.height < 1 || s.cam.grid_width < 1 || s.cam.grid_height < 1)
+        return svo_set_error(SVO_ERR_INVALID, "%s: sequence %d: bad arguments", who, b);
+    const int64_t cells = ((int64_t)(s.width + s.cam.grid_height - 1) / s.cam.grid_height) *
+                          ((int64_t)(s.height + s.cam.grid_width - 1) / s.cam.grid_width);
+    if (cells > s.occupied_count)
+        return svo_set_error(SVO_ERR_INVALID, "%s: sequence %d: %lld merge cells, occupied holds %d", who, b,
+                             (long long)cells, s.occupied_count);
+    if (counts) {
+        int32_t nd[SVO_MAX_PYRAMID_LEVELS], n = 0;
+        if (const int rc = read_i32(s.n_det, n_levels, nd)) return rc;
+        if (const int rc = read_i32(s.kps.n, 1, &n)) return rc;
+        for (int l = 0; l < n_levels; l++)
+            if (nd[l] < 0 || nd[l] > max_cells)
+                return svo_set_error(SVO_ERR_INVALID, "%s: sequence %d: n_det[%d] = %d is outside "
+                                     "0..max_cells = %d", who, b, l, nd[l], max_cells);
+        if (n < 0 || n > cap)
+            return svo_set_error(SVO_ERR_INVALID, "%s: sequence %d: n = %d is outside 0..cap = %d", who, b, n, cap);
+    }
+    memset(&ma, 0, sizeof(ma));
+    ma.cam = s.cam; ma.width = s.width; ma.height = s.height;
+    ma.det = reinterpret_cast<const DetCell*>(s.det); ma.n_det = s.n_det; ma.n_levels = n_levels; ma.max_cells = max_cells;
+    ma.kps = kps_dev(s.kps); ma.cap = cap;
+    ma.sel = reinterpret_cast<DetCell*>(s.sel); ma.sel_level = s.sel_level; ma.sel_cell = s.sel_cell; ma.occupied = s.occupied;
+    ma.old_count = s.old_count; ma.overflow = s.overflow;
+    ma.enable = s.enable;
+    return SVO_OK;
 }
 
 extern "C" int svo_keyframe_merge_batch(svo_handle* h, int batch, const svo_merge_sequence* seqs, int n_levels,
@@ -660,39 +693,72 @@
                              "max_cells >= 1 and cap >= 1", SVO_MAX_PYRAMID_LEVELS);
     HIP_TRY(hipStreamSynchronize(h->stream));
     std::vector<MergeArgs> blocks((size_t)batch);
-    for (int b = 0; b < batch; b++) {
-        const svo_merge_sequence& s = seqs[b];
-        if (planes_missing(s.kps, true) || !s.det || !s.n_det || !s.sel || !s.sel_level || !s.sel_cell || !s.occupied ||
-            !s.old_count || !s.overflow || s.width < 1 || s.height < 1 || s.cam.grid_width < 1 || s.cam.grid_height < 1)
-            return svo_set_error(SVO_ERR_INVALID, "svo_keyframe_merge_batch: sequence %d: bad arguments", b);
-        const int64_t cells = ((int64_t)(s.width + s.cam.grid_height - 1) / s.cam.grid_height) *
-                              ((int64_t)(s.height + s.cam.grid_width - 1) / s.cam.grid_width);
-        if (cells > s.occupied_count)
-            return svo_set_error(SVO_ERR_INVALID, "svo_keyframe_merge_batch: sequence %d: %lld merge cells, occupied holds %d", b,
-                                 (long long)cells, s.occupied_count);
-        int32_t nd[SVO_MAX_PYRAMID_LEVELS], n = 0;
-        if (const int rc = read_i32(s.n_det, n_levels, nd)) return rc;
-        if (const int rc = read_i32(s.kps.n, 1, &n)) return rc;
-        for (int l = 0; l < n_levels; l++)
-            if (nd[l] < 0 || nd[l] > max_cells)
-                return svo_set_error(SVO_ERR_INVALID, "svo_keyframe_merge_batch: sequence %d: n_det[%d] = %d is outside "
-                                     "0..max_cells = %d", b, l, nd[l], max_cells);
-        if (n < 0 || n > cap)
-            return svo_set_error(SVO_ERR_INVALID, "svo_keyframe_merge_batch: sequence %d: n = %d is outside 0..cap = %d", b, n, cap);
-        MergeArgs& ma = blocks[(size_t)b];
-        memset(&ma, 0, sizeof(ma));
-        ma.cam = s.cam; ma.width = s.width; ma.height = s.height;
-        ma.det = reinterpret_cast<const DetCell*>(s.det); ma.n_det = s.n_det; ma.n_levels = n_levels; ma.max_cells = max_cells;
-        ma.kps = kps_dev(s.kps); ma.cap = cap;
-        ma.sel = reinterpret_cast<DetCell*>(s.sel); ma.sel_level = s.sel_level; ma.sel_cell = s.sel_cell; ma.occupied = s.occupied;
-        ma.old_count = s.old_count; ma.overflow = s.overflow;
-        ma.enable = s.enable;
-    }
+    for (int b = 0; b < batch; b++)
+        if (const int rc = fill_merge_args("svo_keyframe_merge_batch", b, seqs[b], n_levels, max_cells, cap, true, blocks[(size_t)b]))
+            return rc;
     MergeArgs* d;
     const int rc = stage(h, blocks, &d);
     if (rc) return rc;
     if (threads) *threads = select_merge_pick_threads(max_cells);
     launch_select_merge(d, batch, max_cells, h->stream);
+    return finish_launch(h);
+}
+
+extern "C" int svo_keyframe_candidates_batch(svo_handle* h, int batch, const svo_keyframe_candidates_sequence* seqs, int n_levels,
+                                             int max_cells, int cap, int skip, uint64_t* skipped) {
+    static const char* who = "svo_keyframe_candidates_batch";
+    CHECK_H(h);
+    if (bad_batch(batch, seqs) || max_cells < 1 || cap < 1 || (skip != 0 && skip != 1))
+        return svo_set_error(SVO_ERR_INVALID, "%s: need 1 <= batch <= 4096, seqs, max_cells >= 1, cap >= 1 and skip 0 or 1", who);
+    HIP_TRY(hipStreamSynchronize(h->stream));
+    std::vector<CompactArgs> cblocks((size_t)batch);
+    std::vector<DetectArgs> dblocks((size_t)batch);
+    std::vector<MergeArgs> mblocks((size_t)batch);
+    const svo_camera_settings& cam0 = seqs[0].merge.cam;
+    int rc = check_detect_levels(who, n_levels, cam0.grid_width, cam0.grid_height);
+    if (rc) return rc;
+    for (int b = 0; b < batch; b++) {
+        const svo_keyframe_candidates_sequence& s = seqs[b];
+        const svo_merge_sequence& m = s.merge;
+        if (s.compact.mode != 1 || s.compact.width != m.width || s.compact.height != m.height || s.compact.zero != m.n_det ||
+            s.compact.zero_count < n_levels || s.compact.dst.kps2d != m.kps.kps2d || s.compact.dst.n != m.kps.n ||
+            m.cam.grid_width != cam0.grid_width || m.cam.grid_height != cam0.grid_height || s.compact.enable || m.enable)
+            return svo_set_error(SVO_ERR_INVALID, "%s: sequence %d: the compaction is mode 1 over the merge's image, clears "
+                                 "its n_det and fills its kps; one cell size for the batch; no enable flags", who, b);
+        if ((rc = fill_compact_args(who, b, s.compact, cap, cblocks[(size_t)b]))) return rc;
+        if ((rc = fill_merge_args(who, b, m, n_levels, max_cells, cap, false, mblocks[(size_t)b]))) return rc;
+        DetectArgs& da = dblocks[(size_t)b];
+        memset(&da, 0, sizeof(da));
+        for (int l = 0; l < n_levels; l++) {
+            const svo_image& im = s.levels[l];
+            int nc;
+            if (!im.data || im.stride < im.width || im.width != (m.width >> l) || im.height != (m.height >> l))
+                return svo_set_error(SVO_ERR_INVALID, "%s: sequence %d: level %d: no data, stride < width, or not the image halved", who, b, l);
+            if ((rc = detect_level_cells(who, l, im.width, im.height, cam0.grid_width, cam0.grid_height, &nc))) return rc;
+            if (nc > max_cells) return svo_set_error(SVO_ERR_CAPACITY, "%s: level %d has %d cells, max_cells = %d", who, l, nc, max_cells);
+            da.level[l] = make_view(im);
+        }
+        da.n_levels = n_levels; da.grid_w = cam0.grid_width; da.grid_h = cam0.grid_height;
+        da.out = const_cast<DetCell*>(mblocks[(size_t)b].det); da.n_out = const_cast<int*>(m.n_det); da.max_cells = max_cells;
+        if (skip) {
+            CompactArgs& ca = cblocks[(size_t)b];
+            ca.occupied = m.occupied; ca.merge_cw = m.cam.grid_height; ca.merge_ch = m.cam.grid_width;
+            ca.skip = m.sel_cell; ca.skip_count = max_cells;
+            ca.skipped = reinterpret_cast<unsigned long long*>(skipped);
+            ca.det = detect_grid(da);
+            da.skip = m.sel_cell;
+            mblocks[(size_t)b].occupied_ready = 1;
+        }
+    }
+    CompactArgs* dc; DetectArgs* dd; MergeArgs* dm;
+    if ((rc = stage(h, cblocks, &dc))) return rc;
+    launch_compact(dc, batch, cap, h->stream);
+    HIP_TRY(hipGetLastError());
+    if ((rc = stage(h, dblocks, &dd))) return rc;
+    launch_detect(dd, batch, max_cells, n_levels, cam0.grid_width, cam0.grid_height, h->stream);
+    HIP_TRY(hipGetLastError());
+    if ((rc = stage(h, mblocks, &dm))) return rc;
+    launch_select_merge(dm, batch, max_cells, h->stream);
     return finish_launch(h);
 }
 
diff --git a/stereo-svo-slam_amd/csrc/svo_ctx.hip b/stereo-svo-slam_amd/csrc/svo_ctx.hip
--- a/stereo-svo-slam_amd/csrc/svo_ctx.hip
+++ b/stereo-svo-slam_amd/csrc/svo_ctx.hip
@@ -1228,6 +1228,18 @@
     return SVO_OK;
 }
 
+extern "C" int svo_ctx_get_detect_skipped(svo_ctx* c, int64_t* cells) {
+    if (!c || !cells) return svo_set_error(SVO_ERR_INVALID, "svo_ctx_get_detect_skipped: bad arguments");
+    int rc = ctx_drain(c);
+    *cells = 0;
+    for (auto& w : c->workers) {
+        int64_t n = 0;
+        if (!rc) rc = grp_detect_skipped(w->g.get(), &n);
+        *cells += n;
+    }
+    return rc;
+}
+
 extern "C" int svo_ctx_get_launch_shapes(svo_ctx* c, svo_launch_shape* out, int max, int* n) {
     if (!c || !n || max < 0 || (max > 0 && !out)) return svo_set_error(SVO_ERR_INVALID, "svo_ctx_get_launch_shapes: bad arguments");
     const int rc = ctx_drain(c);
diff --git a/stereo-svo-slam_amd/csrc/svo_group.hip b/stereo-svo-slam_amd/csrc/svo_group.hip
--- a/stereo-svo-slam_amd/csrc/svo_group.hip
+++ b/stereo-svo-slam_amd/csrc/svo_group.hip
@@ -279,6 +279,7 @@
     alloc(&q.sia_mats, 1); alloc(&q.d_kfs, c->max_kf);
     alloc(&q.det, SVO_MAX_PYRAMID_LEVELS * cells); alloc(&q.n_det, SVO_MAX_PYRAMID_LEVELS);
     alloc(&q.sel, cells); alloc(&q.sel_level, cells); alloc(&q.sel_cell, cells); alloc(&q.occupied, c->merge_cells);
+    alloc(&q.det_skip, cells);
     alloc(&q.color_lcg, 1);
     if (rc) return rc;
     q.kf.init();
@@ -351,6 +352,7 @@
         if ((rc = alloc_sequence(c, c->seqs[s], s))) return rc;
     if ((rc = grow_kf_slabs(c, std::max(2 * n_sequences, 32)))) return rc;
     if ((rc = alloc_template_cache(c))) return rc;
+    if ((rc = dev_alloc(c, &c->d_det_skipped, 1))) return rc;
     if ((rc = alloc_mirrored_table(c, c->remap_img, c->remap_img_host, 2 * (size_t)n_sequences))) return rc;
     HIP_TRY(hipDeviceSynchronize());
     *out = std::move(g);
@@ -378,6 +380,15 @@
 }
 
 const std::vector<svo_launch_shape>& grp_launch_shapes(const svo_group* c) { return c->launch_shapes; }
+
+int grp_detect_skipped(svo_group* c, int64_t* out) {
+    unsigned long long v = 0;
+    HIP_TRY(hipSetDevice(c->device));
+    HIP_TRY(hipMemcpyAsync(&v, c->d_det_skipped, sizeof(v), hipMemcpyDeviceToHost, c->stream.get()));
+    HIP_TRY(hipStreamSynchronize(c->stream.get()));
+    *out = (int64_t)v;
+    return SVO_OK;
+}
 
 namespace svo {
 
diff --git a/stereo-svo-slam_amd/csrc/svo_group.hpp b/stereo-svo-slam_amd/csrc/svo_group.hpp
--- a/stereo-svo-slam_amd/csrc/svo_group.hpp
+++ b/stereo-svo-slam_amd/csrc/svo_group.hpp
@@ -77,3 +77,4 @@
 void grp_enable_timing(svo_group* g, int on);
 svo_totals grp_totals(const svo_group* g);
 const std::vector<svo_launch_shape>& grp_launch_shapes(const svo_group* g);
+int grp_detect_skipped(svo_group* g, int64_t* out);
diff --git a/stereo-svo-slam_amd/csrc/svo_group_state.hpp b/stereo-svo-slam_amd/csrc/svo_group_state.hpp
--- a/stereo-svo-slam_amd/csrc/svo_group_state.hpp
+++ b/stereo-svo-slam_amd/csrc/svo_group_state.hpp
@@ -178,6 +178,7 @@
     int kfs_retired = 0;
     DetCell* det = nullptr; int* n_det = nullptr;
     DetCell* sel = nullptr; int* sel_level = nullptr; int* sel_cell = nullptr; int* occupied = nullptr;
+    int* det_skip = nullptr;
     uint32_t* color_lcg = nullptr;
     std::vector<std::unique_ptr<ImageSet>> sets;
     std::vector<ImageSet*> free_sets;
@@ -248,6 +249,7 @@
     int* h_n = nullptr;
     int* d_n_all = nullptr;
     int* d_inside = nullptr; int* h_inside = nullptr;
+    unsigned long long* d_det_skipped = nullptr;
     size_t readback_bytes = 0;
     uint8_t* d_stage_in = nullptr; size_t stage_frame_bytes = 0;
     const svo::RemapMap* rect = nullptr;
diff --git a/stereo-svo-slam_amd/csrc/svo_group_step.hip b/stereo-svo-slam_amd/csrc/svo_group_step.hip
--- a/stereo-svo-slam_amd/csrc/svo_group_step.hip
+++ b/stereo-svo-slam_amd/csrc/svo_group_step.hip
@@ -352,6 +352,8 @@
     CompactArgs& ca = pack_compact(c, q, slot, 1);
     ca.width = c->width; ca.height = c->height;
     ca.zero = q.n_det; ca.zero_count = SVO_MAX_PYRAMID_LEVELS;
+    ca.occupied = q.occupied; ca.merge_cw = q.cam.grid_height; ca.merge_ch = q.cam.grid_width;
+    ca.skip = q.det_skip; ca.skip_count = c->max_cells; ca.skipped = c->d_det_skipped;
     if (first_frame) {
         ca.start = 1;
         ca.zero_res = reinterpret_cast<int*>(dr); ca.zero_res_count = (int)(sizeof(FrameResult) / sizeof(int));
@@ -360,11 +362,14 @@
     for (int l = 0; l < c->cam.max_pyramid_levels; l++) da.level[l] = q.cur_set->left[l];
     da.n_levels = c->det_levels; da.grid_w = c->cam.grid_width; da.grid_h = c->cam.grid_height;
     da.out = q.det; da.n_out = q.n_det; da.max_cells = c->max_cells;
+    da.skip = q.det_skip;
+    ca.det = detect_grid(da);
     MergeArgs& ma = clear(a.merge.h[slot]);
     ma.cam = q.cam; ma.width = c->width; ma.height = c->height;
     ma.det = q.det; ma.n_det = q.n_det; ma.n_levels = c->det_levels; ma.max_cells = c->max_cells;
     ma.kps = q.kps[q.cur]; ma.cap = c->cap;
     ma.sel = q.sel; ma.sel_level = q.sel_level; ma.sel_cell = q.sel_cell; ma.occupied = q.occupied;
+    ma.occupied_ready = 1;
     ma.old_count = &dr->old_count; ma.overflow = &dr->overflow;
     pack_ssd(c, q, slot, 0, &dr->old_count);
     KfInitArgs& ia = clear(a.kf_init.h[slot]);
@@ -397,7 +402,7 @@
     }
     launch_select_merge(a.merge.d, m, c->max_cells, st);
     HIP_TRY(hipGetLastError());
-    launch_ssd(a.ssd.d, m, c->cap, c->cam.window_size_depth_calculator, c->cam.search_y, st);
+    launch_ssd(a.ssd.d, m, std::min(c->cap, c->max_cells), c->cam.window_size_depth_calculator, c->cam.search_y, st);
     HIP_TRY(hipGetLastError());
     launch_kf_init(a.kf_init.d, m, st);
     HIP_TRY(hipGetLastError());
diff --git a/stereo-svo-slam_amd/csrc/svo_handle.hpp b/stereo-svo-slam_amd/csrc/svo_handle.hpp
--- a/stereo-svo-slam_amd/csrc/svo_handle.hpp
+++ b/stereo-svo-slam_amd/csrc/svo_handle.hpp
@@ -77,6 +77,9 @@
     return SVO_OK;
 }
 
+int check_detect_levels(const char* who, int n_levels, int grid_width, int grid_height);
+int detect_level_cells(const char* who, int l, int width, int height, int grid_width, int grid_height, int* cells);
+
 enum : unsigned {
     KP_KPS2D = 1 << 0, KP_KPS3D = 1 << 1, KP_FLAGS = 1 << 2, KP_KF_ID = 1 << 3, KP_KP_INDEX = 1 << 4, KP_OUTL = 1 << 5,
     KP_INL = 1 << 6, KP_KFX = 1 << 7, KP_KFP = 1 << 8, KP_SCORE = 1 << 9, KP_LEVEL_TYPE = 1 << 10, KP_COLOR = 1 << 11,
diff --git a/stereo-svo-slam_amd/csrc/svo_tracker.hpp b/stereo-svo-slam_amd/csrc/svo_tracker.hpp
--- a/stereo-svo-slam_amd/csrc/svo_tracker.hpp
+++ b/stereo-svo-slam_amd/csrc/svo_tracker.hpp
@@ -35,6 +35,12 @@
     fa.width = width; fa.height = height; fa.inside_count = inside_count;
 }
 
+struct DetectGrid {
+    int n_levels, grid_w, grid_h;
+    int max_cell_w, max_cell_h;
+    int w[SVO_MAX_PYRAMID_LEVELS], h[SVO_MAX_PYRAMID_LEVELS];
+};
+
 struct CompactArgs {
     KpsDev src, dst;
     int mode;
@@ -46,6 +52,12 @@
     int* zero_res;
     int zero_res_count;
     int* min_kf;
+    int* occupied;
+    int merge_cw, merge_ch;
+    int* skip;
+    int skip_count;
+    unsigned long long* skipped;
+    DetectGrid det;
 };
 void launch_compact(const CompactArgs* d_args, int batch, int cap, hipStream_t stream);
 int compact_pick_threads(int cap);
@@ -63,7 +75,9 @@
     int* n_out;
     int max_cells;
     const int* enable;
-};
+    const int* skip;
+};
+DetectGrid detect_grid(const DetectArgs& da);
 void launch_detect(const DetectArgs* d_args, int batch, int max_cells, int n_levels, int grid_w, int grid_h, hipStream_t stream);
 struct DetectShape { int cell_w, cell_h, list; };
 DetectShape detect_pick_shape(int grid_w, int grid_h);
@@ -80,6 +94,7 @@
     int* sel_level;
     int* sel_cell;
     int* occupied;
+    int occupied_ready;
     int* old_count;
     int* overflow;
     const int* enable;
diff --git a/stereo-svo-slam_amd/stereo_svo_slam_amd/hip_lib.py b/stereo-svo-slam_amd/stereo_svo_slam_amd/hip_lib.py
--- a/stereo-svo-slam_amd/stereo_svo_slam_amd/hip_lib.py
+++ b/stereo-svo-slam_amd/stereo_svo_slam_amd/hip_lib.py
@@ -48,7 +48,7 @@
     "svo_keyframe_launch_info", "svo_compact_batch", "svo_keyframe_merge_batch", "svo_keyframe_init_batch",
     "svo_keyframe_record_layout", "svo_ssd_disparity_batch",
     "svo_sparse_align_batch_mats", "svo_pose_mats_layout", "svo_filter_update_table_batch",
-    "svo_sia_records_check",
+    "svo_sia_records_check", "svo_ctx_get_detect_skipped", "svo_keyframe_candidates_batch",
 )
 
 INPUT_GRAY_PAIR, INPUT_BGR_PAIR, INPUT_RGB_PAIR, INPUT_SBS_GRAY, INPUT_SBS_BGR, INPUT_SBS_RGB, INPUT_CH3_ECON = range(7)
@@ -160,6 +160,10 @@
                 ("n_det", C.c_void_p), ("kps", KpsPlanes), ("sel", C.c_void_p), ("sel_level", C.c_void_p),
                 ("sel_cell", C.c_void_p), ("occupied", C.c_void_p), ("old_count", C.c_void_p), ("overflow", C.c_void_p),
                 ("enable", C.c_void_p), ("occupied_count", C.c_int32), ("pad_", C.c_int32)]
+
+
+class KeyframeCandidatesSequence(C.Structure):
+    _fields_ = [("compact", CompactSequence), ("merge", MergeSequence), ("levels", Image * 8)]
 
 
 class KfInitSequence(C.Structure):
@@ -1192,6 +1196,19 @@
                                               C.byref(threads)))
         return threads.value
 
+    def keyframe_candidates_batch(self, seqs, n_levels, max_cells, cap, skip=True):
+        arr = (KeyframeCandidatesSequence * len(seqs))()
+        for a, s in zip(arr, seqs):
+            _fill(a.compact, s["compact"])
+            _fill(a.merge, s["merge"])
+            for l, t in enumerate(s["levels"]):
+                a.levels[l] = _img(t)
+        skipped = torch.zeros(1, dtype=torch.int64, device="cuda")
+        torch.cuda.synchronize()
+        _check(lib().svo_keyframe_candidates_batch(self._h, len(seqs), arr, int(n_levels), int(max_cells), int(cap),
+                                                   int(bool(skip)), _ptr(skipped)))
+        return int(skipped.item())
+
     def keyframe_init_batch(self, seqs, cap):
         arr = (KfInitSequence * len(seqs))()
         for a, s in zip(arr, seqs):
diff --git a/stereo-svo-slam_amd/stereo_svo_slam_amd/stereo_slam.py b/stereo-svo-slam_amd/stereo_svo_slam_amd/stereo_slam.py
--- a/stereo-svo-slam_amd/stereo_svo_slam_amd/stereo_slam.py
+++ b/stereo-svo-slam_amd/stereo_svo_slam_amd/stereo_slam.py
@@ -961,6 +961,11 @@
         _check(lib().svo_get_totals(self._ctx, C.byref(t)))
         return t
 
+    def detect_skipped(self):
+        n = C.c_int64(0)
+        _check(lib().svo_ctx_get_detect_skipped(self._ctx, C.byref(n)))
+        return n.value
+
     def launch_shapes(self):
         n = C.c_int(0)
         _check(lib().svo_ctx_get_launch_shapes(self._ctx, None, 0, C.byref(n)))
```
